# DidItWork/Sigma-Zero

Measured on AMD Instinct MI355X. Metric: MCTS simulations/sec (self-play), higher is better.
Workload: dtype bf16

## Files before the change

### include/sigmazero.h

```cpp
#ifndef SIGMAZERO_H
#define SIGMAZERO_H
#include <stdint.h>

#ifdef __cplusplus
extern "C" {
#endif

#define SZ_RING 256
#define SZ_PLANES 119
#define SZ_ACTIONS 4672
#define SZ_MAX_MOVES 218
#define SZ_POS_BYTES 80

enum {
    SZ_OK = 0,
    SZ_ERR_INVALID = -1,
    SZ_ERR_HIP = -2,
    SZ_ERR_CAPACITY = -3,
    SZ_ERR_NO_DEVICE = -4,
    SZ_ERR_STATE = -5,
    SZ_ERR_ZERO_VISITS = -6
};

enum { SZ_PLANES_F32 = 0, SZ_PLANES_BF16 = 1, SZ_PLANES_NHWC128_BF16 = 2, SZ_PLANES_NHWC128_BITS = 3 };


typedef struct sz_engine sz_engine;

typedef struct sz_config {
    int32_t n_boards;
    int32_t num_searches;
    float   c_puct;
    int32_t learning;
    float   noise_value;
    int32_t chess960;
    int32_t edges_per_board;
    int32_t planes_dtype;
    int32_t device;
    int32_t reuse_subtree;
} sz_config;

typedef struct sz_stats {
    uint64_t simulations;
    uint64_t expansions;
    uint64_t terminal_hits;
    uint64_t sum_depth;
    uint64_t sum_children;
    uint64_t max_edges_used;
    int32_t  boards_pending;
    int32_t  boards_done;
    int32_t  boards_error;
    int32_t  first_error;
} sz_stats;

int sz_create(const sz_config* cfg, sz_engine** out);
int sz_destroy(sz_engine* e);

int sz_new_games(sz_engine* e, const int32_t* scharnagl, const uint8_t* active, void* stream);

int sz_upload_game(sz_engine* e, int32_t board, const void* ring, int32_t ply, void* stream);
int sz_set_active(sz_engine* e, const uint8_t* active, void* stream);

int sz_compact(sz_engine* e, int32_t enable, int32_t* n_live_out, void* stream);

int sz_search_begin(sz_engine* e, void* planes_dev, void* stream);

int sz_search_step(sz_engine* e, const float* policy_dev, const float* value_dev, void* planes_dev, void* stream);

int sz_get_stats(sz_engine* e, sz_stats* out, void* stream);

int sz_root_children(sz_engine* e, int32_t* action_dev, int32_t* visits_dev, int32_t* n_child_dev,
                     float* prior_dev, double* value_sum_dev, void* stream);

int sz_play(sz_engine* e, const double* uniforms_dev, void* stream);

int sz_fetch_ply(sz_engine* e, uint8_t* packed_planes, int32_t* action, int32_t* visits, int32_t* n_child,
                 uint8_t* colour, int32_t* chosen, uint8_t* game_over, int8_t* result, uint8_t* active, void* stream);

int sz_set_root_noise(sz_engine* e, const float* gamma_dev);

int sz_debug_step_stamps(sz_engine* e, void* dev_buffer);

int sz_debug_pending(sz_engine* e, uint64_t* mask, int32_t* depth, int32_t* n_nodes, int32_t* n_edges,
                     int32_t* status, void* stream);
int sz_debug_tree(sz_engine* e, int32_t board, int32_t max_nodes, int32_t* depth, int32_t* action, int32_t* visits, double* value_sum,
                  float* prior, int32_t* n_out, void* stream);
int sz_debug_select(const int32_t* offsets_dev, const int32_t* vc_dev, const double* value_sum_dev, const float* prior_dev,
                    const int32_t* parent_visits_dev, const float* c_dev, float* ucb_out_dev, int32_t* argmax_out_dev, int32_t n_cases, void* stream);
int sz_debug_position(sz_engine* e, int32_t board, void* pos_out, int32_t* ply, void* stream);


int sz_nn_conv_bf16(const void* in, const void* w_packed, const float* bias, const void* residual, void* out,
                    int32_t n_boards, int32_t cin, int32_t ksize, int32_t relu, void* stream);
#define SZ_NN_W16 0x40000
#define SZ_NN_IN_BITS 0x1000000
int sz_nn_block_bf16(const void* in, const void* w1_packed, const float* bias1, const void* w2_packed, const float* bias2, void* out,
                     int32_t n_boards, int32_t flags, void* stream);
int sz_nn_pack_weights(const float* w_in, int32_t cin_real, int32_t cin_padded, int32_t ksize, uint16_t* out);

int sz_nn_pack_weights16(const float* w_in, int32_t cin_real, int32_t cin_padded, int32_t ksize, uint16_t* out);
#define SZ_NN_F16 0x8000000
int sz_nn_pack_weights16_f16(const float* w_in, int32_t cin_real, int32_t cin_padded, int32_t ksize, uint16_t* out);
int sz_nn_pack_head16_f16(const float* w_in, uint16_t* out);

#define SZ_NN_TOWER_WGB1 0x10000000
#define SZ_NN_TOWER_WGB2 0x20000000
int sz_nn_tower_bf16(const void* planes, const void* const* w_packed, const float* const* bias, int32_t n_blocks, void* out,
                     int32_t n_boards, int32_t flags , void* stream);
#define SZ_NN_SPLIT_WGB1 0x2000000
#define SZ_NN_SPLIT_WGB2 0x4000000
int sz_nn_tower_split(const void* planes, const void* w_stream, const float* bias, int32_t n_blocks, float* out,
                      int32_t n_boards, int32_t flags , void* stream);
int64_t sz_nn_split_stream_elems(int32_t n_blocks);
int sz_nn_pack_split_stream(const float* w_in, int32_t cin_real, int32_t ksize , int32_t conv, uint16_t* stream);
int sz_nn_forward_split(const void* planes, const void* w_stream, const float* bias, int32_t n_blocks, const void* w_p2_packed, const float* b_p2,
                        const float* wv, float bv, const float* fc1_w_t, const float* fc1_b, const float* fc2_w, float fc2_b, float* probs, float* value,
                        float* v1_scratch, float* tower_out, int32_t n_boards, int32_t do_softmax, int32_t flags, void* stream);
int sz_nn_pack_split_head(const float* w_in , uint16_t* out);
int sz_nn_pack_split_stream_f16(const float* w_in, int32_t cin_real, int32_t ksize, int32_t conv, uint16_t* stream);
int sz_nn_pack_split_head_f16(const float* w_in, uint16_t* out);
int sz_nn_conv3x3_split_f32(const float* x, const void* w_stream, const float* zero256, float* y, int32_t n_boards, int32_t f16, void* amax_bits, void* stream);
int sz_nn_wgrad3x3_split_f32(const float* gy, const float* x, const void* amax_gy, const void* amax_x, float* part, float* dw, int32_t n_boards, void* stream);
int sz_nn_pack_conv_split_dev(const float* w, int32_t transposed, int32_t f16, void* w_stream, void* zero_u32 , void* stream);
int sz_nn_pack_conv_split_both(const float* w, int32_t f16, void* w_stream, void* w_stream_t, void* zero_u32, void* stream);
int sz_nn_conv3x3_train_fwd(const float* x, const float* w, int32_t f16, void* w_stream, void* w_stream_t, const float* zero256, float* y, int32_t n_boards, void* amax2, void* stream);
int sz_nn_conv3x3_train_bwd(const float* gy, const float* x, const void* w_stream_t, const float* zero256, float* gx, void* amax2, float* part, float* dw, int32_t n_boards,
                            int32_t f16, void* stream);
int sz_bn_act_train_fwd(const float* x, const float* gamma, const float* beta, float* running_mean, float* running_var, float momentum, float eps, const float* residual,
                        float* y, float* save_mean, float* save_invstd, int32_t n_boards, int32_t channels, void* stream);
int sz_bn_act_train_bwd(const float* gy, const float* x, const float* y, const float* gamma, const float* save_mean, const float* save_invstd, float* dx, float* dres,
                        float* dgamma, float* dbeta, int32_t n_boards, int32_t channels, void* stream);
int sz_nn_value_mlp(const float* v1, const float* fc1_w_t, const float* fc1_b, const float* fc2_w, float fc2_b, float* value, int32_t n_boards, void* stream);
int sz_nn_debug_split_stamps(void* dev_buffer, int32_t mode );
int sz_nn_debug_tower_stamps(void* dev_buffer, int32_t mode );
int sz_debug_stream_read(const void* src, uint64_t bytes, int32_t mode, void* sink16, void* stream);
int sz_nn_policy_head_bf16(const void* t, const void* w_packed, const float* bias, float* probs, int32_t n_boards, int32_t do_softmax, void* stream);
int sz_nn_value_head_bf16(const void* x, const float* wv, float bv, const float* fc1_w_t, const float* fc1_b, const float* fc2_w, float fc2_b,
                          float* value, int32_t n_boards, void* stream);
int sz_nn_pack_head16(const float* w_in, uint16_t* out);
int sz_nn_heads_bf16(const void* x, const void* w_p1_packed, const float* b_p1, const void* w_p2_packed, const float* b_p2, const float* wv, float bv,
                     const float* fc1_w_t, const float* fc1_b, const float* fc2_w, float fc2_b, float* probs, float* value, float* v1_scratch,
                     int32_t n_boards, int32_t do_softmax, void* stream);

const char* sz_error_string(int code);
int sz_device_count(void);


typedef struct szh_game szh_game;

szh_game* szh_game_new(int chess960, int scharnagl);
szh_game* szh_game_from_fen(const char* fen, int chess960);
szh_game* szh_game_copy(const szh_game* g);
void      szh_game_free(szh_game* g);
int  szh_legal_actions(const szh_game* g, int32_t* idx);
int  szh_action_to_move(const szh_game* g, int idx, int32_t* from, int32_t* to, int32_t* promo);
int  szh_move_to_action(int from, int to, int promo, int white);
int  szh_push_action(szh_game* g, int idx);
int  szh_push_move(szh_game* g, int from, int to, int promo);
void szh_status(const szh_game* g, int32_t* out12);
void szh_planes(const szh_game* g, uint8_t* out );
uint64_t szh_perft(szh_game* g, int depth);
void szh_bitboards(const szh_game* g, uint64_t* out10);
int  szh_export(const szh_game* g, void* ring_out, int32_t* ply, int32_t* chess960);
int  szh_is_chess960(const szh_game* g);
int  szh_plane_bits_mismatches(const szh_game* g);

#ifdef __cplusplus
}
#endif
#endif
```

### sigma-zero_amd/_native.py

```python
import ctypes as C
import os

from . import build as _build

SZ_RING, SZ_PLANES, SZ_ACTIONS, SZ_MAX_MOVES, SZ_POS_BYTES, SZ_MASK_WORDS = 256, 119, 4672, 218, 80, 73
SZ_OK, SZ_ERR_INVALID, SZ_ERR_HIP, SZ_ERR_CAPACITY, SZ_ERR_NO_DEVICE, SZ_ERR_STATE, SZ_ERR_ZERO_VISITS = 0, -1, -2, -3, -4, -5, -6
SZ_PLANES_F32, SZ_PLANES_BF16, SZ_PLANES_NHWC128_BF16, SZ_PLANES_NHWC128_BITS = 0, 1, 2, 3
SZ_NN_W16 = 0x40000
SZ_NN_IN_BITS = 0x1000000
SZ_NN_SPLIT_WGB1, SZ_NN_SPLIT_WGB2 = 0x2000000, 0x4000000
SZ_NN_F16 = 0x8000000
SZ_NN_TOWER_WGB1, SZ_NN_TOWER_WGB2 = 0x10000000, 0x20000000


class sz_config(C.Structure):
    _fields_ = [("n_boards", C.c_int32), ("num_searches", C.c_int32), ("c_puct", C.c_float), ("learning", C.c_int32),
                ("noise_value", C.c_float), ("chess960", C.c_int32), ("edges_per_board", C.c_int32),
                ("planes_dtype", C.c_int32), ("device", C.c_int32), ("reuse_subtree", C.c_int32)]


class sz_stats(C.Structure):
    _fields_ = [("simulations", C.c_uint64), ("expansions", C.c_uint64), ("terminal_hits", C.c_uint64), ("sum_depth", C.c_uint64),
                ("sum_children", C.c_uint64), ("max_edges_used", C.c_uint64), ("boards_pending", C.c_int32),
                ("boards_done", C.c_int32), ("boards_error", C.c_int32), ("first_error", C.c_int32)]


class NativeError(RuntimeError):
    def __init__(self, code, what=""):
        self.code = code
        msg = lib().sz_error_string(code).decode() if _lib is not None else str(code)
        super().__init__("sigmazero native call failed%s: %s (%d)" % (" in " + what if what else "", msg, code))


EXPORTS = {
    "sz_create": (C.c_int, [C.POINTER(sz_config), C.POINTER(C.c_void_p)]),
    "sz_destroy": (C.c_int, [C.c_void_p]),
    "sz_new_games": (C.c_int, [C.c_void_p, C.c_void_p, C.c_void_p, C.c_void_p]),
    "sz_upload_game": (C.c_int, [C.c_void_p, C.c_int32, C.c_void_p, C.c_int32, C.c_void_p]),
    "sz_set_active": (C.c_int, [C.c_void_p, C.c_void_p, C.c_void_p]),
    "sz_compact": (C.c_int, [C.c_void_p, C.c_int32, C.POINTER(C.c_int32), C.c_void_p]),
    "sz_search_begin": (C.c_int, [C.c_void_p, C.c_void_p, C.c_void_p]),
    "sz_search_step": (C.c_int, [C.c_void_p, C.c_void_p, C.c_void_p, C.c_void_p, C.c_void_p]),
    "sz_get_stats": (C.c_int, [C.c_void_p, C.POINTER(sz_stats), C.c_void_p]),
    "sz_root_children": (C.c_int, [C.c_void_p] + [C.c_void_p] * 5 + [C.c_void_p]),
    "sz_play": (C.c_int, [C.c_void_p, C.c_void_p, C.c_void_p]),
    "sz_fetch_ply": (C.c_int, [C.c_void_p] + [C.c_void_p] * 9 + [C.c_void_p]),
    "sz_debug_pending": (C.c_int, [C.c_void_p] + [C.c_void_p] * 5 + [C.c_void_p]),
    "sz_debug_position": (C.c_int, [C.c_void_p, C.c_int32, C.c_void_p, C.POINTER(C.c_int32), C.c_void_p]),
    "sz_debug_tree": (C.c_int, [C.c_void_p, C.c_int32, C.c_int32] + [C.c_void_p] * 5 + [C.POINTER(C.c_int32), C.c_void_p]),
    "sz_debug_select": (C.c_int, [C.c_void_p] * 8 + [C.c_int32, C.c_void_p]),
    "sz_nn_conv_bf16": (C.c_int, [C.c_void_p] * 5 + [C.c_int32] * 4 + [C.c_void_p]),
    "sz_nn_block_bf16": (C.c_int, [C.c_void_p] * 6 + [C.c_int32] * 2 + [C.c_void_p]),
    "sz_nn_tower_bf16": (C.c_int, [C.c_void_p, C.c_void_p, C.c_void_p, C.c_int32, C.c_void_p, C.c_int32, C.c_int32, C.c_void_p]),
    "sz_nn_tower_split": (C.c_int, [C.c_void_p, C.c_void_p, C.c_void_p, C.c_int32, C.c_void_p, C.c_int32, C.c_int32, C.c_void_p]),
    "sz_nn_debug_split_stamps": (C.c_int, [C.c_void_p, C.c_int32]),
    "sz_nn_split_stream_elems": (C.c_int64, [C.c_int32]),
    "sz_nn_pack_split_stream": (C.c_int, [C.c_void_p, C.c_int32, C.c_int32, C.c_int32, C.c_void_p]),
    "sz_nn_forward_split": (C.c_int, [C.c_void_p, C.c_void_p, C.c_void_p, C.c_int32, C.c_void_p, C.c_void_p, C.c_void_p, C.c_float, C.c_void_p, C.c_void_p, C.c_void_p, C.c_float,
                                      C.c_void_p, C.c_void_p, C.c_void_p, C.c_void_p, C.c_int32, C.c_int32, C.c_int32, C.c_void_p]),
    "sz_nn_pack_split_head": (C.c_int, [C.c_void_p, C.c_void_p]),
    "sz_nn_pack_split_head_f16": (C.c_int, [C.c_void_p, C.c_void_p]),
    "sz_nn_pack_split_stream_f16": (C.c_int, [C.c_void_p, C.c_int32, C.c_int32, C.c_int32, C.c_void_p]),
    "sz_nn_conv3x3_split_f32": (C.c_int, [C.c_void_p, C.c_void_p, C.c_void_p, C.c_void_p, C.c_int32, C.c_int32, C.c_void_p, C.c_void_p]),
    "sz_nn_wgrad3x3_split_f32": (C.c_int, [C.c_void_p, C.c_void_p, C.c_void_p, C.c_void_p, C.c_void_p, C.c_void_p, C.c_int32, C.c_void_p]),
    "sz_nn_pack_conv_split_dev": (C.c_int, [C.c_void_p, C.c_int32, C.c_int32, C.c_void_p, C.c_void_p, C.c_void_p]),
    "sz_nn_pack_conv_split_both": (C.c_int, [C.c_void_p, C.c_int32, C.c_void_p, C.c_void_p, C.c_void_p, C.c_void_p]),
    "sz_bn_act_train_fwd": (C.c_int, [C.c_void_p, C.c_void_p, C.c_void_p, C.c_void_p, C.c_void_p, C.c_float, C.c_float, C.c_void_p, C.c_void_p, C.c_void_p, C.c_void_p, C.c_int32, C.c_int32, C.c_void_p]),
    "sz_bn_act_train_bwd": (C.c_int, [C.c_void_p, C.c_void_p, C.c_void_p, C.c_void_p, C.c_void_p, C.c_void_p, C.c_void_p, C.c_void_p, C.c_void_p, C.c_void_p, C.c_int32, C.c_int32, C.c_void_p]),
    "sz_nn_conv3x3_train_fwd": (C.c_int, [C.c_void_p, C.c_void_p, C.c_int32, C.c_void_p, C.c_void_p, C.c_void_p, C.c_void_p, C.c_int32, C.c_void_p, C.c_void_p]),
    "sz_nn_conv3x3_train_bwd": (C.c_int, [C.c_void_p, C.c_void_p, C.c_void_p, C.c_void_p, C.c_void_p, C.c_void_p, C.c_void_p, C.c_void_p, C.c_int32, C.c_int32, C.c_void_p]),
    "sz_nn_value_mlp": (C.c_int, [C.c_void_p, C.c_void_p, C.c_void_p, C.c_void_p, C.c_float, C.c_void_p, C.c_int32, C.c_void_p]),
    "sz_debug_stream_read": (C.c_int, [C.c_void_p, C.c_uint64, C.c_int32, C.c_void_p, C.c_void_p]),
    "sz_nn_policy_head_bf16": (C.c_int, [C.c_void_p] * 4 + [C.c_int32] * 2 + [C.c_void_p]),
    "sz_debug_step_stamps": (C.c_int, [C.c_void_p, C.c_void_p]),
    "sz_set_root_noise": (C.c_int, [C.c_void_p, C.c_void_p]),
    "sz_nn_debug_tower_stamps": (C.c_int, [C.c_void_p, C.c_int32]),
    "sz_nn_heads_bf16": (C.c_int, [C.c_void_p] * 6 + [C.c_float] + [C.c_void_p] * 3 + [C.c_float] + [C.c_void_p] * 3 + [C.c_int32] * 2 + [C.c_void_p]),
    "sz_nn_value_head_bf16": (C.c_int, [C.c_void_p, C.c_void_p, C.c_float, C.c_void_p, C.c_void_p, C.c_void_p, C.c_float, C.c_void_p, C.c_int32, C.c_void_p]),
    "sz_nn_pack_head16": (C.c_int, [C.c_void_p, C.c_void_p]),
    "sz_nn_pack_head16_f16": (C.c_int, [C.c_void_p, C.c_void_p]),
    "sz_nn_pack_weights16_f16": (C.c_int, [C.c_void_p, C.c_int32, C.c_int32, C.c_int32, C.c_void_p]),
    "sz_nn_pack_weights16": (C.c_int, [C.c_void_p, C.c_int32, C.c_int32, C.c_int32, C.c_void_p]),
    "sz_nn_pack_weights": (C.c_int, [C.c_void_p, C.c_int32, C.c_int32, C.c_int32, C.c_void_p]),
    "sz_error_string": (C.c_char_p, [C.c_int]),
    "sz_device_count": (C.c_int, []),
    "szh_game_new": (C.c_void_p, [C.c_int, C.c_int]),
    "szh_game_from_fen": (C.c_void_p, [C.c_char_p, C.c_int]),
    "szh_game_copy": (C.c_void_p, [C.c_void_p]),
    "szh_game_free": (None, [C.c_void_p]),
    "szh_legal_actions": (C.c_int, [C.c_void_p, C.POINTER(C.c_int32)]),
    "szh_action_to_move": (C.c_int, [C.c_void_p, C.c_int, C.POINTER(C.c_int32), C.POINTER(C.c_int32), C.POINTER(C.c_int32)]),
    "szh_move_to_action": (C.c_int, [C.c_int, C.c_int, C.c_int, C.c_int]),
    "szh_push_action": (C.c_int, [C.c_void_p, C.c_int]),
    "szh_push_move": (C.c_int, [C.c_void_p, C.c_int, C.c_int, C.c_int]),
    "szh_status": (None, [C.c_void_p, C.POINTER(C.c_int32)]),
    "szh_planes": (None, [C.c_void_p, C.c_void_p]),
    "szh_perft": (C.c_uint64, [C.c_void_p, C.c_int]),
    "szh_bitboards": (None, [C.c_void_p, C.POINTER(C.c_uint64)]),
    "szh_export": (C.c_int, [C.c_void_p, C.c_void_p, C.POINTER(C.c_int32), C.POINTER(C.c_int32)]),
    "szh_is_chess960": (C.c_int, [C.c_void_p]),
    "szh_plane_bits_mismatches": (C.c_int, [C.c_void_p]),
}

_lib = None


def lib():
    global _lib
    if _lib is not None:
        return _lib
    path = _build.LIB
    if not os.path.exists(path):
        raise RuntimeError("libsigmazero_hip.so is not built (%s). Run: python -c \"import __graft_entry__ as g; g.build()\". "
                           "The search path has no CPU fallback." % path)
    L = C.CDLL(path)
    for name, (res, args) in EXPORTS.items():
        fn = getattr(L, name)
        fn.restype, fn.argtypes = res, args
    _lib = L
    return L


def check(code, what=""):
    if code != SZ_OK:
        raise NativeError(code, what)
```

### sigma-zero_amd/csrc/sz_nn_split.hip

```cpp
#include "sz_nn_common.h"

#define NN_MAX_CONVS_SPLIT 129
#ifndef SP_PF
#define SP_PF 1
#endif
#define SP_WSCALE_LOG2 10
#ifndef SP_EXPLICIT_WAIT
#define SP_EXPLICIT_WAIT 1
#endif
#define SP_RING (SP_PF == 1 ? 2 : 4)
#define SP_KSTEP_U4 2048

template <int WGB> struct SplitGeom {
    static constexpr int PITCH = NN_COUT * 2 + NN_PAD16;
    static constexpr int IMG = WGB * 64 * PITCH + NN_ZERO16;
    static constexpr int NJ = 4 * WGB;
    static constexpr int TAB = 2 * IMG;
    static constexpr int SCR = 2 * IMG + 9 * NJ * 64 * 4;
    static constexpr int LDS_BYTES = SCR + 1024;
    static constexpr int PITCH_IN = 128 * 2 + NN_PAD16;
};

template <int CIN, int WGB, bool BLO, bool TAB, int ABL = 0 ,
          int NTAPS = 9 ,
          class E = ElemBF16 ,
          int NI = 4 >
__device__ __forceinline__ void split_kloop(const unsigned char* lds, const int offH, const int offL, const int* addr_tab, const WSrc& wr,
                                            const uint32_t ks_base, const uint32_t ks_after, const float* __restrict__ bias,
                                            f32x4 (&acc)[NI][4 * WGB], uint4 (&ring)[SP_RING][2 * NI], const int co_tile0 = -1 ) {
    constexpr int PITCH = CIN * 2 + NN_PAD16;
    constexpr int KSTEPS = CIN / 32;
    constexpr int NJ = 4 * WGB, G = WGB;
    constexpr int NPROD = BLO ? 3 : 2;
    constexpr bool SKIPROWS = WGB == 2 && NN_ROWSKIP && NTAPS == 9;
    static_assert(NTAPS == 9 || NTAPS == 1, "3x3 or 1x1");
    static_assert(KSTEPS % SP_RING == 0, "ring slots must be compile-time indices");
    static_assert(8 + 2 * NI <= NPROD * NI * 3, "every memory instruction needs an MFMA gap of its own");
    int lane = threadIdx.x & 63;
    asm volatile("" : "+v"(lane));
    const int wave = threadIdx.x >> 6;
    const int p16 = lane & 15, kg = lane >> 4;
    const int ct0 = co_tile0 < 0 ? wave * NI : co_tile0;
    const uint32_t wlane = (uint32_t)(ct0 * 64 + lane) * 16u;
    {
        f32x4 binit[NI];
#pragma unroll
        for (int i = 0; i < NI; i++) binit[i] = *(const f32x4*)(bias + (ct0 + i) * 16 + 4 * kg);
#pragma unroll
        for (int i = 0; i < NI; i++)
#pragma unroll
            for (int j = 0; j < NJ; j++) acc[i][j] = binit[i];
    }
    constexpr int TABPITCH = NN_COUT * 2 + NN_PAD16;
    auto tap_addr = [&](int tap, int j) -> int {
        if constexpr (TAB) {
            const int rel = addr_tab[((NTAPS == 1 ? 4 : tap) * NJ + j) * 64 + lane];
            if constexpr (PITCH == TABPITCH) return rel;
            else {
                const int row = (int)__umulhi((unsigned)rel, 7895161u);
                return rel >= WGB * 64 * TABPITCH ? rel - WGB * 64 * (TABPITCH - PITCH) : rel - row * (TABPITCH - PITCH);
            }
        } else return conv_tap_addr16<PITCH, NTAPS, WGB>(tap, j, p16, kg);
    };
    const int lds_base = (int)(uint32_t)(uintptr_t)lds;
    auto abs_addr = [&](int rel) -> int {
        int a = lds_base + offH + rel;
        asm volatile("" : "+v"(a));
        return a;
    };
    auto LD = [](int addr) -> bf16x8 { return *(const __attribute__((address_space(3))) bf16x8*)(uint32_t)addr; };
    int bcurH[NJ], bcurL[BLO ? NJ : 1], bnxt[NJ];
    bf16x8 bH[2][4], bL[4];
#pragma unroll
    for (int j = 0; j < NJ; j++) {
        bnxt[j] = tap_addr(0, j);
        bcurH[j] = abs_addr(bnxt[j]);
        if constexpr (BLO) bcurL[j] = bcurH[j] + (offL - offH);
    }
#pragma unroll
    for (int m = 0; m < 4; m++)
        if (!(SKIPROWS && m == 0)) bH[0][m] = LD(bcurH[m]);
    auto tap_body = [&](const int tap, auto skip_tag) {
        constexpr int SK = decltype(skip_tag)::value;
        if (tap + 1 < NTAPS) {
#pragma unroll
            for (int j = 0; j < NJ; j++) bnxt[j] = tap_addr(tap + 1, j);
        }
#pragma unroll
        for (int kc = 0; kc < KSTEPS; kc++) {
            const int slot = kc & (SP_RING - 1);
            const uint32_t ks_next = (kc + SP_PF >= KSTEPS && tap == NTAPS - 1) ? ks_after + (uint32_t)(kc + SP_PF - KSTEPS) : ks_base + (uint32_t)(tap * KSTEPS + kc + SP_PF);
#pragma unroll
            for (int g = 0; g < G; g++) {
                const int buf = (kc * G + g) & 1;
#pragma unroll
                for (int prod = 0; prod < NPROD; prod++) {
#pragma unroll
                    for (int i = 0; i < NI; i++) {
                        const bf16x8 a = __builtin_bit_cast(bf16x8, ring[slot][prod == 1 ? NI + i : i]);
#pragma unroll
                        for (int m = 0; m < 4; m++) {
                            const bool idle_g = SKIPROWS && ((SK == 1 && g == 0) || (SK == 2 && g == G - 1));
                            const bool idle = idle_g && m == (SK == 1 ? 0 : 3);
                            if (idle) continue;
                            acc[i][g * 4 + m] = E::mfma(a, prod == 2 ? bL[m] : bH[buf][m], acc[i][g * 4 + m]);
                            const int NR = idle_g ? 3 : 4, q = (prod * NI + i) * NR + (idle_g && SK == 1 ? m - 1 : m);
                            if (q < 4) {
                                if constexpr (BLO && !(ABL & 2)) {
                                    const bool idl = SKIPROWS && ((SK == 1 && g == 0 && q == 0) || (SK == 2 && g == G - 1 && q == 3));
                                    if (!idl) bL[q] = LD(bcurL[g * 4 + q] + kc * 64);
                                }
                            } else if (q < 8) {
                                const int mm = q - 4;
                                if (ABL & 2) {
                                } else if (g + 1 < G) {
                                    if (!(SKIPROWS && SK == 2 && g + 1 == G - 1 && mm == 3)) bH[buf ^ 1][mm] = LD(bcurH[(g + 1) * 4 + mm] + kc * 64);
                                } else if (kc + 1 < KSTEPS) {
                                    if (!(SKIPROWS && SK == 1 && mm == 0)) bH[buf ^ 1][mm] = LD(bcurH[mm] + (kc + 1) * 64);
                                } else if (tap + 1 < NTAPS) {
                                    if (!(SKIPROWS && mm == 0 && tap + 1 < 3)) bH[buf ^ 1][mm] = LD(abs_addr(bnxt[mm]));
                                }
                            } else if (q < 8 + 2 * NI && g == 0) {
                                const int f = q - 8;
                                if (!(ABL & 1)) ring[(kc + SP_PF) & (SP_RING - 1)][f] = ld_wfrag(wr, (size_t)ks_next * SP_KSTEP_U4 + (f >= NI ? SP_KSTEP_U4 / 2 : 0), wlane + (f % NI) * 1024);
                            }
#if SP_EXPLICIT_WAIT
                            if (q == 2 * NI * NR - 1 && NPROD == 3) __builtin_amdgcn_s_waitcnt(0xC07F);
                            if (q == NPROD * NI * NR - 1) {
                                if (g == G - 1) __builtin_amdgcn_s_waitcnt(0x0070 | ((SP_PF - 1) * 2 * NI));
                                else __builtin_amdgcn_s_waitcnt(0xC07F);
                            }
#endif
                            asm volatile("" ::: "memory");
                            __builtin_amdgcn_sched_barrier(0);
                        }
                    }
                }
            }
        }
        if (NTAPS > 1) {
#pragma unroll
            for (int j = 0; j < NJ; j++) {
                bcurH[j] = abs_addr(bnxt[j]);
                if constexpr (BLO) bcurL[j] = bcurH[j] + (offL - offH);
            }
        }
    };
    using SK0 = std::integral_constant<int, 0>;
    if constexpr (SKIPROWS) {
        using SK1 = std::integral_constant<int, 1>; using SK2 = std::integral_constant<int, 2>;
        for (int tap = 0; tap < 3; tap++) tap_body(tap, SK1{});
        for (int tap = 3; tap < 6; tap++) tap_body(tap, SK0{});
        for (int tap = 6; tap < 9; tap++) tap_body(tap, SK2{});
    } else {
        for (int tap = 0; tap < NTAPS; tap++) tap_body(tap, SK0{});
    }
}

__device__ __forceinline__ float to_agpr(float v) { float a; asm volatile("v_accvgpr_write_b32 %0, %1" : "=a"(a) : "v"(v)); return a; }
__device__ __forceinline__ float from_agpr(float a) { float v; asm volatile("v_accvgpr_read_b32 %0, %1" : "=v"(v) : "a"(a)); return v; }
__device__ __forceinline__ float relu_f32(float v) { const int i = __builtin_bit_cast(int, v); return __builtin_bit_cast(float, i > 0 ? i : 0); }

template <int WGB, int MODE, class E = ElemBF16>
__device__ __forceinline__ void split_epilogue(unsigned char* hi_img, unsigned char* lo_img, const f32x4 (&acc)[4][4 * WGB], float (&xres)[4][4 * WGB][4]) {
    constexpr bool SCALED = std::is_same<E, ElemF16>::value;
    constexpr float USC = 1.0f / (float)(1 << SP_WSCALE_LOG2);
    constexpr int PITCH = NN_COUT * 2 + NN_PAD16;
    int lane = threadIdx.x & 63;
    asm volatile("" : "+v"(lane));
    const int wave = threadIdx.x >> 6;
    const int p16 = lane & 15, kg = lane >> 4;
#pragma unroll
    for (int j = 0; j < 4 * WGB; j++) {
        const int row = tile_row<WGB>(j, p16);
        const int rowoff = row * PITCH, g = (row >> 2) & 1;
#pragma unroll
        for (int ip = 0; ip < 4; ip += 2) {
            uint2 h[2], l[2];
            float r[2][4];
            f32x4 v[2];
#pragma unroll
            for (int d = 0; d < 2; d++)
#pragma unroll
                for (int k = 0; k < 4; k++) r[d][k] = MODE == 2 ? from_agpr(xres[ip + d][j][k]) : 0.f;
#pragma unroll
            for (int d = 0; d < 2; d++) {
                v[d] = acc[ip + d][j];
#pragma unroll
                for (int k = 0; k < 4; k++) {
                    if (SCALED) v[d][k] *= USC;
                    if (MODE == 2) v[d][k] += r[d][k];
                    v[d][k] = relu_f32(v[d][k]);
                }
            }
#pragma unroll
            for (int d = 0; d < 2; d++)
#pragma unroll
                for (int k = 0; k < 4; k++)
                    if (MODE != 1) xres[ip + d][j][k] = to_agpr(v[d][k]);
#pragma unroll
            for (int d = 0; d < 2; d++) {
                h[d].x = E::pack2(v[d][0], v[d][1]); h[d].y = E::pack2(v[d][2], v[d][3]);
                l[d].x = E::pack2(v[d][0] - E::lo(h[d].x), v[d][1] - E::hi(h[d].x));
                l[d].y = E::pack2(v[d][2] - E::lo(h[d].y), v[d][3] - E::hi(h[d].y));
            }
            const auto hx = __builtin_amdgcn_permlane16_swap(h[0].x, h[1].x, false, false), hy = __builtin_amdgcn_permlane16_swap(h[0].y, h[1].y, false, false);
            const auto lx = __builtin_amdgcn_permlane16_swap(l[0].x, l[1].x, false, false), ly = __builtin_amdgcn_permlane16_swap(l[0].y, l[1].y, false, false);
            const int it = ip + (kg & 1);
            const int chunk = ((wave * 4 + it) * 16 + 4 * (kg & 2)) >> 3;
            const int off = rowoff + ((chunk ^ g) << 4);
            *(uint4*)(hi_img + off) = make_uint4(hx[0], hy[0], hx[1], hy[1]);
            *(uint4*)(lo_img + off) = make_uint4(lx[0], ly[0], lx[1], ly[1]);
        }
    }
}

struct SplitHeadsParams {
    const uint4* w_p2;
    const float* b_p2;
    const float* wv;
    float bv;
    float* probs;
    float* v1_out;
    int do_softmax;
};

template <int WGB, class E = ElemBF16>
__device__ __forceinline__ void split_heads_tail(unsigned char* lds, const int* addr_tab, const WSrc& wr, const uint32_t ks_p1, const float* __restrict__ bias_p1,
                                                 const SplitHeadsParams& hp, f32x4 (&acc)[4][4 * WGB], uint4 (&ring)[SP_RING][8], float (&xres)[4][4 * WGB][4],
                                                 const int board0, const int n_boards) {
    using GEO = SplitGeom<WGB>;
    constexpr int NJ = GEO::NJ, NT = WGB, PITCH = GEO::PITCH;
    unsigned char* imgH = lds;
    unsigned char* imgL = lds + GEO::IMG;
    float* psum = (float*)(lds + GEO::SCR);
    float* red = psum + WGB * 64;
    int lane = threadIdx.x & 63;
    asm volatile("" : "+v"(lane));
    const int wave = threadIdx.x >> 6, p16 = lane & 15, kg = lane >> 4;
    {
        const int row = wave * 64 + lane;
        if (row < WGB * 64) {
            const unsigned char* ph = imgH + row * PITCH;
            const unsigned char* pl = imgL + row * PITCH;
            const int g = (row >> 2) & 1;
            float sv = 0.f;
#pragma unroll 4
            for (int c8 = 0; c8 < 32; c8++) {
                const uint4 h = *(const uint4*)(ph + ((c8 ^ g) << 4)), l = *(const uint4*)(pl + ((c8 ^ g) << 4));
                const float4 w0 = ((const float4*)hp.wv)[c8 * 2], w1 = ((const float4*)hp.wv)[c8 * 2 + 1];
                sv = __builtin_fmaf(w0.x, E::lo(h.x) + E::lo(l.x), sv); sv = __builtin_fmaf(w0.y, E::hi(h.x) + E::hi(l.x), sv);
                sv = __builtin_fmaf(w0.z, E::lo(h.y) + E::lo(l.y), sv); sv = __builtin_fmaf(w0.w, E::hi(h.y) + E::hi(l.y), sv);
                sv = __builtin_fmaf(w1.x, E::lo(h.z) + E::lo(l.z), sv); sv = __builtin_fmaf(w1.y, E::hi(h.z) + E::hi(l.z), sv);
                sv = __builtin_fmaf(w1.z, E::lo(h.w) + E::lo(l.w), sv); sv = __builtin_fmaf(w1.w, E::hi(h.w) + E::hi(l.w), sv);
            }
            const int board = board0 + (row >> 6);
            if (board < n_boards) hp.v1_out[(size_t)board * 64 + (row & 63)] = fmaxf(sv + hp.bv, 0.f);
        }
    }
    split_kloop<256, WGB, true, true, 0, 1, E>(lds, 0, GEO::IMG, addr_tab, wr, ks_p1, 0u, bias_p1, acc, ring);
    __syncthreads();
    split_epilogue<WGB, 1, E>(imgH, imgL, acc, xres);
    __syncthreads();
    f32x4 pa[5][NT];
#pragma unroll
    for (int i = 0; i < 5; i++)
#pragma unroll
        for (int t = 0; t < NT; t++) pa[i][t] = f32x4{0.f, 0.f, 0.f, 0.f};
    int baddr[NT];
#pragma unroll
    for (int t = 0; t < NT; t++) baddr[t] = addr_tab[(4 * NJ + wave * NT + t) * 64 + lane];
#pragma unroll 2
    for (int kc = 0; kc < 8; kc++) {
        bf16x8 ah[5], al[5], bh[NT], bl[NT];
#pragma unroll
        for (int i = 0; i < 5; i++) {
            ah[i] = __builtin_bit_cast(bf16x8, hp.w_p2[(size_t)(kc * 10 + i) * 64 + lane]);
            al[i] = __builtin_bit_cast(bf16x8, hp.w_p2[(size_t)(kc * 10 + 5 + i) * 64 + lane]);
        }
#pragma unroll
        for (int t = 0; t < NT; t++) { bh[t] = *(const bf16x8*)(imgH + baddr[t] + kc * 64); bl[t] = *(const bf16x8*)(imgL + baddr[t] + kc * 64); }
#pragma unroll
        for (int prod = 0; prod < 3; prod++)
#pragma unroll
            for (int i = 0; i < 5; i++)
#pragma unroll
                for (int t = 0; t < NT; t++)
                    pa[i][t] = E::mfma(prod == 1 ? al[i] : ah[i], prod == 2 ? bl[t] : bh[t], pa[i][t]);
    }
    __syncthreads();
    float mx = -3.0e38f;
#pragma unroll
    for (int i = 0; i < 5; i++)
#pragma unroll
        for (int r = 0; r < 4; r++) {
            const int co = i * 16 + 4 * kg + r;
            const float bb = co < 73 ? hp.b_p2[co] : 0.f;
#pragma unroll
            for (int t = 0; t < NT; t++) {
                if (std::is_same<E, ElemF16>::value) pa[i][t][r] *= 1.0f / (float)(1 << SP_WSCALE_LOG2);
                pa[i][t][r] += bb;
                if (co < 73) mx = fmaxf(mx, pa[i][t][r]);
            }
        }
    const int lboard = WGB == 2 ? (p16 >> 3) : 0;
    float inv = 1.0f;
    if (hp.do_softmax) {
        mx = fmaxf(mx, __shfl_xor(mx, 1)); mx = fmaxf(mx, __shfl_xor(mx, 2)); mx = fmaxf(mx, __shfl_xor(mx, 4));
        if (WGB == 1) mx = fmaxf(mx, __shfl_xor(mx, 8));
        mx = fmaxf(mx, __shfl_xor(mx, 16)); mx = fmaxf(mx, __shfl_xor(mx, 32));
        if ((lane & (WGB == 2 ? 0x37 : 0x3F)) == 0) red[wave * 2 + lboard] = mx;
        __syncthreads();
        mx = fmaxf(fmaxf(red[0 + lboard], red[2 + lboard]), fmaxf(red[4 + lboard], red[6 + lboard]));
#pragma unroll
        for (int t = 0; t < NT; t++) {
            float ps = 0.f;
#pragma unroll
            for (int i = 0; i < 5; i++)
#pragma unroll
                for (int r = 0; r < 4; r++) {
                    const int co = i * 16 + 4 * kg + r;
                    const float e = co < 73 ? __expf(pa[i][t][r] - mx) : 0.f;
                    pa[i][t][r] = e;
                    ps += e;
                }
            ps += __shfl_xor(ps, 16);
            ps += __shfl_xor(ps, 32);
            const int row = tile_row<WGB>(wave * NT + t, p16);
            if (kg == 0) psum[row] = ps;
        }
        __syncthreads();
        float tot = 0.f;
#pragma unroll 8
        for (int p = 0; p < 64; p++) tot += psum[lboard * 64 + p];
        inv = 1.0f / tot;
    }
    if (board0 + lboard < n_boards) {
        float* pb = hp.probs + (size_t)(board0 + lboard) * 4672;
#pragma unroll
        for (int t = 0; t < NT; t++) {
            const int pos = tile_row<WGB>(wave * NT + t, p16) & 63;
#pragma unroll
            for (int i = 0; i < 5; i++)
#pragma unroll
                for (int r = 0; r < 4; r++) {
                    const int co = i * 16 + 4 * kg + r;
                    if (co < 73) pb[co * 64 + pos] = pa[i][t][r] * inv;
                }
        }
    }
}

#define SPSTAMP(k) do { if (MODE != 0 && stamp_now) { unsigned long long _t = __builtin_amdgcn_s_memtime(); if ((threadIdx.x & 63) == 0) stamps[(size_t)(blockIdx.x * 4 + (threadIdx.x >> 6)) * 16 + (k)] = _t; } } while (0)
template <int WGB, int MODE, bool HEADS, class E = ElemBF16>
__global__ __launch_bounds__(256, 1) void k_tower_split(const uint16_t* __restrict__ planes, const uint4* __restrict__ wstream, const float* __restrict__ bias,
                                                         float* __restrict__ out, int n_boards, int n_blocks, int flags, unsigned long long* __restrict__ stamps,
                                                         const SplitHeadsParams hp) {
    constexpr int ABL = MODE >= 2 ? MODE - 1 : 0;
    using GEO = SplitGeom<WGB>;
    constexpr int NJ = GEO::NJ;
    extern __shared__ __attribute__((aligned(16))) unsigned char lds[];
    unsigned char* imgH = lds;
    unsigned char* imgL = lds + GEO::IMG;
    for (int c = threadIdx.x; c < NN_ZERO16 / 16; c += 256) {
        *(uint4*)(imgH + WGB * 64 * GEO::PITCH + c * 16) = make_uint4(0, 0, 0, 0);
        *(uint4*)(imgL + WGB * 64 * GEO::PITCH + c * 16) = make_uint4(0, 0, 0, 0);
    }
    int* addr_tab = (int*)(lds + GEO::TAB);
    for (int e = threadIdx.x; e < 9 * NJ * 64; e += 256)
        addr_tab[e] = conv_tap_addr16<GEO::PITCH, 9, WGB, true>(e / (NJ * 64), (e >> 6) % NJ, e & 15, (e >> 4) & 3);
    const int lane = threadIdx.x & 63, wave = threadIdx.x >> 6;
    const int n_tiles = (n_boards + WGB - 1) / WGB;
    const int n_convs = 1 + 2 * n_blocks;
    const WSrc wr = wfrag_rsrc(wstream);
    f32x4 acc[4][NJ];
    float xres[4][NJ][4];
    uint4 ring[SP_RING][8];
    {
        const uint32_t wlane = (uint32_t)((wave * 4) * 64 + lane) * 16u;
#pragma unroll
        for (int k = 0; k < SP_PF; k++)
#pragma unroll
            for (int f = 0; f < 8; f++) ring[k][f] = ld_wfrag(wr, (size_t)k * SP_KSTEP_U4 + (f >= 4 ? SP_KSTEP_U4 / 2 : 0), wlane + (f & 3) * 1024);
    }
    for (int tile = blockIdx.x; tile < n_tiles; tile += gridDim.x) {
        const int board0 = tile * WGB;
        if (flags & SZ_NN_IN_BITS) stage_tile_bits<WGB, NN_PAD16, E, true>(imgL, planes, board0, n_boards);
        else stage_tile<128, WGB, NN_PAD16, false, true>(imgL, planes, board0, n_boards, false);
        __syncthreads();
        uint32_t ks = 0;
        const uint32_t ks_p1 = 36u + 72u * (uint32_t)(n_convs - 1);
        const uint32_t ks_end = HEADS ? ks_p1 : 0u;
        split_kloop<128, WGB, false, true, 0, 9, E>(lds, GEO::IMG, GEO::IMG, addr_tab, wr, ks, n_convs > 1 ? 36u : ks_end, bias, acc, ring);
        ks += 36;
        __syncthreads();
        split_epilogue<WGB, 0, E>(imgH, imgL, acc, xres);
        __syncthreads();
        for (int c = 1; c < n_convs; c++) {
            const bool stamp_now = MODE != 0 && (c == 7 || c == 8) && tile == (int)(blockIdx.x + gridDim.x);
            const int sb = (c & 1) ? 0 : 5;
            SPSTAMP(sb + 0);
            split_kloop<256, WGB, true, true, ABL, 9, E>(lds, 0, GEO::IMG, addr_tab, wr, ks, c + 1 < n_convs ? ks + 72u : ks_end, bias + c * NN_COUT, acc, ring);
            ks += 72;
            SPSTAMP(sb + 1);
            __syncthreads();
            SPSTAMP(sb + 2);
            if (c & 1) split_epilogue<WGB, 1, E>(imgH, imgL, acc, xres);
            else split_epilogue<WGB, 2, E>(imgH, imgL, acc, xres);
            SPSTAMP(sb + 3);
            __syncthreads();
            SPSTAMP(sb + 4);
            if (MODE != 0 && stamp_now && c == 8 && (threadIdx.x & 63) == 0) stamps[(size_t)(blockIdx.x * 4 + (threadIdx.x >> 6)) * 16 + 10] = __builtin_amdgcn_s_memrealtime();
        }
        if constexpr (HEADS) split_heads_tail<WGB, E>(lds, addr_tab, wr, ks_p1, bias + n_convs * NN_COUT, hp, acc, ring, xres, board0, n_boards);
        const int p16 = lane & 15, kg = lane >> 4;
        if (!HEADS || out)
#pragma unroll
        for (int j = 0; j < NJ; j++) {
            const int row = tile_row<WGB>(j, p16);
            if (board0 + (row >> 6) < n_boards) {
                float* dst = out + ((size_t)board0 * 64 + row) * NN_COUT;
#pragma unroll
                for (int i = 0; i < 4; i++)
                    *(f32x4*)(dst + (wave * 4 + i) * 16 + 4 * kg) = f32x4{from_agpr(xres[i][j][0]), from_agpr(xres[i][j][1]), from_agpr(xres[i][j][2]), from_agpr(xres[i][j][3])};
            }
        }
    }
}

#ifndef SZ_CONV_ABL
#define SZ_CONV_ABL 0
#endif
template <class E, int COSPLIT>
__global__ __launch_bounds__(256, 1) void k_conv3x3_split_f32(const float* __restrict__ x, const uint4* __restrict__ wstream, const float* __restrict__ zero_bias,
                                                               float* __restrict__ y, int n_boards, unsigned int* __restrict__ amax_bits ) {
    constexpr int WGB = 1;
    constexpr bool SCALED = std::is_same<E, ElemF16>::value;
    using GEO = SplitGeom<WGB>;
    constexpr int NJ = GEO::NJ, PITCH = GEO::PITCH, NI = 4 / COSPLIT;
    extern __shared__ __attribute__((aligned(16))) unsigned char lds[];
    unsigned char* imgH = lds;
    unsigned char* imgL = lds + GEO::IMG;
    float* wmax = (float*)(lds + GEO::SCR);
    for (int c = threadIdx.x; c < NN_ZERO16 / 16; c += 256) {
        *(uint4*)(imgH + WGB * 64 * PITCH + c * 16) = make_uint4(0, 0, 0, 0);
        *(uint4*)(imgL + WGB * 64 * PITCH + c * 16) = make_uint4(0, 0, 0, 0);
    }
    int* addr_tab = (int*)(lds + GEO::TAB);
    for (int e = threadIdx.x; e < 9 * NJ * 64; e += 256)
        addr_tab[e] = conv_tap_addr16<PITCH, 9, WGB, true>(e / (NJ * 64), (e >> 6) % NJ, e & 15, (e >> 4) & 3);
    const int lane = threadIdx.x & 63, wave = threadIdx.x >> 6;
    const WSrc wr = wfrag_rsrc(wstream);
    f32x4 acc[NI][NJ];
    uint4 ring[SP_RING][2 * NI];
    const int half = COSPLIT == 2 ? (int)(blockIdx.x & 1) : 0, ct0 = half * 8 + wave * NI;
    {
        const uint32_t wlane = (uint32_t)(ct0 * 64 + lane) * 16u;
#pragma unroll
        for (int k = 0; k < SP_PF; k++)
#pragma unroll
            for (int f = 0; f < 2 * NI; f++) ring[k][f] = ld_wfrag(wr, (size_t)k * SP_KSTEP_U4 + (f >= NI ? SP_KSTEP_U4 / 2 : 0), wlane + (f % NI) * 1024);
    }
    for (int board = blockIdx.x / COSPLIT; board < n_boards; board += gridDim.x / COSPLIT) {
        __syncthreads();
        const float4* src = (const float4*)(x + (size_t)board * 256 * 64);
        float4 v[16];
#pragma unroll
        for (int t = 0; t < 16; t++) v[t] = src[(wave + 4 * t) * 64 + lane];
        float sx = 1.f, unscale = 1.f;
        if (SCALED) {
            float m = 0.f;
#pragma unroll
            for (int t = 0; t < 16; t++) m = fmaxf(fmaxf(m, fmaxf(fabsf(v[t].x), fabsf(v[t].y))), fmaxf(fabsf(v[t].z), fabsf(v[t].w)));
            for (int off = 32; off >= 1; off >>= 1) m = fmaxf(m, __shfl_xor(m, off));
            if (lane == 0) wmax[wave] = m;
            __syncthreads();
            m = fmaxf(fmaxf(wmax[0], wmax[1]), fmaxf(wmax[2], wmax[3]));
            if (amax_bits && threadIdx.x == 0 && half == 0) atomicMax(amax_bits, __builtin_bit_cast(unsigned int, m));
            const int ex = (int)((__builtin_bit_cast(uint32_t, m) >> 23) & 0xFF);
            const int k = (ex == 0 || ex == 255) ? 0 : 11 - (ex - 127);
            const int kc = k < -100 ? -100 : (k > 100 ? 100 : k);
            sx = __builtin_bit_cast(float, (uint32_t)(127 + kc) << 23);
            unscale = __builtin_bit_cast(float, (uint32_t)(127 - kc - SP_WSCALE_LOG2) << 23);
        }
#pragma unroll
        for (int t = 0; t < 16; t++) {
            const int q = wave + 4 * t;
            const int c = q * 4 + (lane >> 4), p0 = (lane & 15) * 4;
            const float vv[4] = {v[t].x * sx, v[t].y * sx, v[t].z * sx, v[t].w * sx};
#pragma unroll
            for (int k = 0; k < 4; k++) {
                const int row = p0 + k;
                const int off = row * PITCH + (((c >> 3) ^ ((row >> 2) & 1)) << 4) + (c & 7) * 2;
                const uint32_t hb = E::pack2(vv[k], 0.f) & 0xFFFFu;
                const uint32_t lb = E::pack2(vv[k] - E::lo(hb), 0.f) & 0xFFFFu;
                if (!(SZ_CONV_ABL & 2) || hb == 0x1234u) {
                    *(uint16_t*)(imgH + off) = (uint16_t)hb;
                    *(uint16_t*)(imgL + off) = (uint16_t)lb;
                }
            }
        }
        __syncthreads();
        if (SZ_CONV_ABL & 1) {
#pragma unroll
            for (int i = 0; i < NI; i++)
#pragma unroll
                for (int j = 0; j < NJ; j++) acc[i][j] = f32x4{sx, sx, sx, sx};
        } else
        split_kloop<256, WGB, true, true, 0, 9, E, NI>(lds, 0, GEO::IMG, addr_tab, wr, 0u, 0u, zero_bias, acc, ring, ct0);
        float* dst = y + (size_t)board * 256 * 64;
        const int p16 = lane & 15, kg = lane >> 4;
#pragma unroll
        for (int i = 0; i < NI; i++)
#pragma unroll
            for (int j = 0; j < NJ; j++)
#pragma unroll
                for (int r = 0; r < ((SZ_CONV_ABL & 4) ? 1 : 4); r++) dst[(size_t)((ct0 + i) * 16 + 4 * kg + r) * 64 + j * 16 + p16] = SCALED ? acc[i][j][r] * unscale : acc[i][j][r];
    }
}

template <class E>
__global__ __launch_bounds__(256) void k_pack_conv_split(const float* __restrict__ w, uint16_t* __restrict__ stream, int transposed, unsigned int* __restrict__ zero_u32,
                                                         uint16_t* __restrict__ stream_t ) {
    int idx = blockIdx.x * 256 + threadIdx.x;
    if (zero_u32 && idx == 0) { zero_u32[0] = 0u; if (stream_t) zero_u32[1] = 0u; }
    if (stream_t && idx >= 72 * 16 * 64 * 8) { idx -= 72 * 16 * 64 * 8; stream = stream_t; transposed = 1; }
    if (idx >= 72 * 16 * 64 * 8) return;
    const int e = idx & 7, l = (idx >> 3) & 63, tile = (idx >> 9) & 15, ks = idx >> 13;
    const int tap = ks >> 3, k32 = ks & 7;
    const int co = tile * 16 + (l & 15), ci = k32 * 32 + 8 * (l >> 4) + e;
    float v = transposed ? w[((size_t)ci * 256 + co) * 9 + (8 - tap)] : w[((size_t)co * 256 + ci) * 9 + tap];
    if (std::is_same<E, ElemF16>::value) v *= (float)(1 << SP_WSCALE_LOG2);
    const uint32_t h = E::pack2(v, 0.f) & 0xFFFFu;
    const uint32_t lo = E::pack2(v - E::lo(h), 0.f) & 0xFFFFu;
    uint16_t* rec = stream + (size_t)ks * SP_KSTEP_U4 * 8;
    rec[((size_t)tile * 64 + l) * 8 + e] = (uint16_t)h;
    rec[(size_t)SP_KSTEP_U4 * 4 + ((size_t)tile * 64 + l) * 8 + e] = (uint16_t)lo;
}

#define WG_ROWPITCH 512
#define WG_TILE_BYTES (10 * WG_ROWPITCH)
#define WG_LDS_BYTES (3 * 4 * WG_TILE_BYTES)
__device__ __forceinline__ float pow2_from_amax_bits(unsigned int bits, int target_log2, int* k_out) {
    const int ex = (int)((bits >> 23) & 0xFF);
    int k = (ex == 0 || ex == 255) ? 0 : target_log2 - (ex - 127);
    k = k < -100 ? -100 : (k > 100 ? 100 : k);
    *k_out = k;
    return __builtin_bit_cast(float, (uint32_t)(127 + k) << 23);
}
__global__ __launch_bounds__(256, 1) void k_wgrad3x3_split(const float* __restrict__ gy, const float* __restrict__ x, const unsigned int* __restrict__ amax_gy,
                                                            const unsigned int* __restrict__ amax_x, float* __restrict__ part, int n_boards, int KG) {
    using E = ElemF16;
    extern __shared__ __attribute__((aligned(16))) unsigned char lds[];
    const int cob = blockIdx.x & 3, cib = (blockIdx.x >> 2) & 3, kgrp = blockIdx.x >> 4;
    const int chunk = (n_boards + KG - 1) / KG, b0 = kgrp * chunk, b1 = min(n_boards, b0 + chunk);
    const int lane = threadIdx.x & 63, wave = threadIdx.x >> 6, wr = wave >> 1, wc = wave & 1;
    const int n = lane & 15, kg = lane >> 4;
    int kgy, kx;
    const float sgy = pow2_from_amax_bits(*amax_gy, 11, &kgy), sx = pow2_from_amax_bits(*amax_x, 11, &kx);
    const float unscale_g = __builtin_bit_cast(float, (uint32_t)(127 - kgy) << 23), unscale_x = __builtin_bit_cast(float, (uint32_t)(127 - kx) << 23);
    for (int c = threadIdx.x; c < WG_LDS_BYTES / 16; c += 256) *(uint4*)(lds + c * 16) = make_uint4(0, 0, 0, 0);
    f32x4 acc[2][2][9];
#pragma unroll
    for (int a = 0; a < 2; a++)
#pragma unroll
        for (int c = 0; c < 2; c++)
#pragma unroll
            for (int t = 0; t < 9; t++) acc[a][c][t] = f32x4{0.f, 0.f, 0.f, 0.f};
    const int sci = threadIdx.x & 63, sq = threadIdx.x >> 6;
    const int sbase = (sci >> 4) * WG_TILE_BYTES + (sci & 15) * 16;
    float4 xq[4], gq[2][2][2];
    auto load_board = [&](int bb) {
        const float4* src = (const float4*)(x + ((size_t)bb * 256 + cib * 64 + sci) * 64 + sq * 16);
#pragma unroll
        for (int i = 0; i < 4; i++) xq[i] = src[i];
#pragma unroll
        for (int cot = 0; cot < 2; cot++)
#pragma unroll
            for (int kh = 0; kh < 2; kh++) {
                const int co = cob * 64 + (2 * wr + cot) * 16 + n;
                const float4* g = (const float4*)(gy + ((size_t)bb * 256 + co) * 64 + (4 * kh + kg) * 8);
                gq[cot][kh][0] = g[0]; gq[cot][kh][1] = g[1];
            }
    };
    if (b0 < b1) load_board(b0);
    for (int b = b0; b < b1; b++) {
        __syncthreads();
        {
            const float4 v0 = xq[0], v1 = xq[1], v2 = xq[2], v3 = xq[3];
            const float rows[2][8] = {{v0.x, v0.y, v0.z, v0.w, v1.x, v1.y, v1.z, v1.w}, {v2.x, v2.y, v2.z, v2.w, v3.x, v3.y, v3.z, v3.w}};
#pragma unroll
            for (int rr = 0; rr < 2; rr++) {
                uint32_t h[8], l[8];
#pragma unroll
                for (int c = 0; c < 8; c++) {
                    const float sv = rows[rr][c] * sx;
                    h[c] = E::pack2(sv, 0.f) & 0xFFFFu;
                    l[c] = E::pack2(sv - E::lo(h[c]), 0.f) & 0xFFFFu;
                }
                const int row = 2 * sq + rr + 1;
#pragma unroll
                for (int dxi = 0; dxi < 3; dxi++) {
                    uint32_t ph[4], pl[4];
#pragma unroll
                    for (int p = 0; p < 4; p++) {
                        const int c0 = 2 * p + dxi - 1, c1 = c0 + 1;
                        ph[p] = ((c0 >= 0 && c0 < 8) ? h[c0] : 0u) | (((c1 >= 0 && c1 < 8) ? h[c1] : 0u) << 16);
                        pl[p] = ((c0 >= 0 && c0 < 8) ? l[c0] : 0u) | (((c1 >= 0 && c1 < 8) ? l[c1] : 0u) << 16);
                    }
                    unsigned char* dst = lds + dxi * 4 * WG_TILE_BYTES + sbase + row * WG_ROWPITCH;
                    *(uint4*)dst = make_uint4(ph[0], ph[1], ph[2], ph[3]);
                    *(uint4*)(dst + 256) = make_uint4(pl[0], pl[1], pl[2], pl[3]);
                }
            }
        }
        bf16x8 ah[2][2], al[2][2];
#pragma unroll
        for (int cot = 0; cot < 2; cot++)
#pragma unroll
            for (int kh = 0; kh < 2; kh++) {
                const float4 g0 = gq[cot][kh][0], g1 = gq[cot][kh][1];
                const float f[8] = {g0.x * sgy, g0.y * sgy, g0.z * sgy, g0.w * sgy, g1.x * sgy, g1.y * sgy, g1.z * sgy, g1.w * sgy};
                uint32_t hh[4], ll[4];
#pragma unroll
                for (int p = 0; p < 4; p++) {
                    hh[p] = E::pack2(f[2 * p], f[2 * p + 1]);
                    ll[p] = E::pack2(f[2 * p] - E::lo(hh[p]), f[2 * p + 1] - E::hi(hh[p]));
                }
                ah[cot][kh] = __builtin_bit_cast(bf16x8, make_uint4(hh[0], hh[1], hh[2], hh[3]));
                al[cot][kh] = __builtin_bit_cast(bf16x8, make_uint4(ll[0], ll[1], ll[2], ll[3]));
            }
        if (b + 1 < b1) load_board(b + 1);
        __syncthreads();
        constexpr int WG_AHEAD = 2, NGRP = 36;
        bf16x8 bh[WG_AHEAD + 1], bl[WG_AHEAD + 1];
        auto fetch = [&](int g) {
            const int kh = g / 18, cit = (g / 9) & 1, tap = g % 9, dy = tap / 3 - 1, dxi = tap % 3;
            const unsigned char* src = lds + (dxi * 4 + 2 * wc + cit) * WG_TILE_BYTES + (4 * kh + kg + dy + 1) * WG_ROWPITCH + n * 16;
            bh[g % (WG_AHEAD + 1)] = *(const bf16x8*)src; bl[g % (WG_AHEAD + 1)] = *(const bf16x8*)(src + 256);
        };
#pragma unroll
        for (int g = 0; g < WG_AHEAD; g++) fetch(g);
#pragma unroll
        for (int g = 0; g < NGRP; g++) {
            if (g + WG_AHEAD < NGRP) fetch(g + WG_AHEAD);
            asm volatile("" ::: "memory");
            __builtin_amdgcn_sched_barrier(0);
            const int kh = g / 18, cit = (g / 9) & 1, tap = g % 9, sl = g % (WG_AHEAD + 1);
#pragma unroll
            for (int cot = 0; cot < 2; cot++) {
                acc[cot][cit][tap] = E::mfma(ah[cot][kh], bh[sl], acc[cot][cit][tap]);
                acc[cot][cit][tap] = E::mfma(al[cot][kh], bh[sl], acc[cot][cit][tap]);
                acc[cot][cit][tap] = E::mfma(ah[cot][kh], bl[sl], acc[cot][cit][tap]);
            }
            asm volatile("" ::: "memory");
            __builtin_amdgcn_sched_barrier(0);
        }
    }
#pragma unroll
    for (int cot = 0; cot < 2; cot++)
#pragma unroll
        for (int cit = 0; cit < 2; cit++)
#pragma unroll
            for (int tap = 0; tap < 9; tap++)
#pragma unroll
                for (int r = 0; r < 4; r++) {
                    const int co = cob * 64 + (2 * wr + cot) * 16 + 4 * kg + r, ci = cib * 64 + (2 * wc + cit) * 16 + n;
                    part[(((size_t)kgrp * 9 + tap) * 256 + co) * 256 + ci] = acc[cot][cit][tap][r] * unscale_g * unscale_x;
                }
}
__global__ __launch_bounds__(256) void k_wgrad_reduce(const float* __restrict__ part, float* __restrict__ dw, int KG) {
    const int idx = blockIdx.x * 256 + threadIdx.x;
    float s[9];
#pragma unroll
    for (int t = 0; t < 9; t++) s[t] = 0.f;
    for (int k = 0; k < KG; k++)
#pragma unroll
        for (int t = 0; t < 9; t++) s[t] += part[((size_t)k * 9 + t) * 65536 + idx];
#pragma unroll
    for (int t = 0; t < 9; t++) dw[(size_t)idx * 9 + t] = s[t];
}

static unsigned long long* g_split_stamps = nullptr;
static int g_split_mode = 1;

extern "C" {

int sz_nn_debug_split_stamps(void* dev_buffer, int32_t mode) { g_split_stamps = (unsigned long long*)dev_buffer; g_split_mode = mode; return SZ_OK; }

int64_t sz_nn_split_stream_elems(int32_t n_blocks) {
    if (n_blocks < 0) return SZ_ERR_INVALID;
    return (int64_t)(36 + 72 * 2 * (int64_t)n_blocks + 8) * SP_KSTEP_U4 * 8;
}

static int pack_split_stream_impl(const float* w_in, int32_t cin_real, int32_t ksize, int32_t conv, uint16_t* stream, bool f16);
int sz_nn_pack_split_stream(const float* w_in, int32_t cin_real, int32_t ksize, int32_t conv, uint16_t* stream) { return pack_split_stream_impl(w_in, cin_real, ksize, conv, stream, false); }
int sz_nn_pack_split_stream_f16(const float* w_in, int32_t cin_real, int32_t ksize, int32_t conv, uint16_t* stream) { return pack_split_stream_impl(w_in, cin_real, ksize, conv, stream, true); }
}
static int pack_split_stream_impl(const float* w_in, int32_t cin_real, int32_t ksize, int32_t conv, uint16_t* stream, bool f16) {
    if (!w_in || !stream || conv < 0 || conv > NN_MAX_CONVS_SPLIT || (ksize != 1 && ksize != 3) || (ksize == 1 && !(conv & 1))) return SZ_ERR_INVALID;
    const int cin_padded = conv == 0 ? 128 : 256, taps = ksize * ksize;
    if (cin_real <= 0 || cin_real > cin_padded) return SZ_ERR_INVALID;
    const int ksteps = cin_padded / 32;
    const size_t ks0 = conv == 0 ? 0 : 36 + (size_t)(conv - 1) * 72;
    const float wscale = f16 ? (float)(1 << SP_WSCALE_LOG2) : 1.f;
    auto rne = [f16](float v) -> uint16_t { return f16 ? ElemF16::from_float(v) : ElemBF16::from_float(v); };
    auto back = [f16](uint16_t h) -> float { if (f16) { _Float16 x; memcpy(&x, &h, 2); return (float)x; } const uint32_t hu = (uint32_t)h << 16; float hf; memcpy(&hf, &hu, 4); return hf; };
    for (int t = 0; t < taps; t++)
        for (int k = 0; k < ksteps; k++) {
            uint16_t* rec = stream + (ks0 + (size_t)t * ksteps + k) * SP_KSTEP_U4 * 8;
            for (int tile = 0; tile < 16; tile++)
                for (int l = 0; l < 64; l++)
                    for (int e = 0; e < 8; e++) {
                        const int co = tile * 16 + (l & 15), ci = k * 32 + 8 * (l >> 4) + e;
                        const float v = (ci < cin_real ? w_in[((size_t)co * cin_real + ci) * taps + t] : 0.f) * wscale;
                        const uint16_t h = rne(v);
                        rec[((size_t)tile * 64 + l) * 8 + e] = h;
                        rec[(size_t)SP_KSTEP_U4 * 4 + ((size_t)tile * 64 + l) * 8 + e] = rne(v - back(h));
                    }
        }
    return SZ_OK;
}
extern "C" {

static int pack_split_head_impl(const float* w_in, uint16_t* out, bool f16);
int sz_nn_pack_split_head(const float* w_in, uint16_t* out) { return pack_split_head_impl(w_in, out, false); }
int sz_nn_pack_split_head_f16(const float* w_in, uint16_t* out) { return pack_split_head_impl(w_in, out, true); }
}
static int pack_split_head_impl(const float* w_in, uint16_t* out, bool f16) {
    if (!w_in || !out) return SZ_ERR_INVALID;
    const float wscale = f16 ? (float)(1 << SP_WSCALE_LOG2) : 1.f;
    auto rne = [f16](float v) -> uint16_t { return f16 ? ElemF16::from_float(v) : ElemBF16::from_float(v); };
    auto back = [f16](uint16_t h) -> float { if (f16) { _Float16 x; memcpy(&x, &h, 2); return (float)x; } const uint32_t hu = (uint32_t)h << 16; float hf; memcpy(&hf, &hu, 4); return hf; };
    for (int ks = 0; ks < 8; ks++)
        for (int tile = 0; tile < 5; tile++)
            for (int l = 0; l < 64; l++)
                for (int e = 0; e < 8; e++) {
                    const int co = tile * 16 + (l & 15), ci = ks * 32 + 8 * (l >> 4) + e;
                    const float v = (co < 73 ? w_in[(size_t)co * 256 + ci] : 0.f) * wscale;
                    const uint16_t h = rne(v);
                    out[((((size_t)ks * 2 + 0) * 5 + tile) * 64 + l) * 8 + e] = h;
                    out[((((size_t)ks * 2 + 1) * 5 + tile) * 64 + l) * 8 + e] = rne(v - back(h));
                }
    return SZ_OK;
}
extern "C" {

}

static int launch_split_one(const void* planes, const void* w_stream, const float* bias, int32_t n_blocks, float* out, int32_t n_boards, int32_t flags, void* stream,
                            const SplitHeadsParams* heads);
static int launch_split(const void* planes, const void* w_stream, const float* bias, int32_t n_blocks, float* out, int32_t n_boards, int32_t flags, void* stream,
                        const SplitHeadsParams* heads) {
    const int n_cu = device_cus(), rem = n_boards % (2 * n_cu);
    if (n_boards > 2 * n_cu && rem > 0 && rem <= n_cu && !(flags & (SZ_NN_SPLIT_WGB1 | SZ_NN_SPLIT_WGB2)) && !g_split_stamps) {
        const int head = n_boards - rem;
        const size_t plane_bytes = (flags & SZ_NN_IN_BITS) ? 64 * sizeof(uint4) : (size_t)64 * 128 * 2;
        const int rc = launch_split_one(planes, w_stream, bias, n_blocks, out, head, flags | SZ_NN_SPLIT_WGB2, stream, heads);
        if (rc != SZ_OK) return rc;
        SplitHeadsParams hp2;
        if (heads) { hp2 = *heads; hp2.probs += (size_t)head * 4672; hp2.v1_out += (size_t)head * 64; }
        return launch_split_one((const unsigned char*)planes + head * plane_bytes, w_stream, bias, n_blocks, out ? out + (size_t)head * 64 * 256 : nullptr, rem,
                                flags | SZ_NN_SPLIT_WGB1, stream, heads ? &hp2 : nullptr);
    }
    return launch_split_one(planes, w_stream, bias, n_blocks, out, n_boards, flags, stream, heads);
}
static int launch_split_one(const void* planes, const void* w_stream, const float* bias, int32_t n_blocks, float* out, int32_t n_boards, int32_t flags, void* stream,
                            const SplitHeadsParams* heads) {
    static bool attr_flags[NN_MAX_DEVICES] = {};
    bool& attr_set = attr_flags[current_device_slot()];
    if (!attr_set) {
#define SPLIT_ATTR(W, M, H) HIPCHK(hipFuncSetAttribute((const void*)k_tower_split<W, M, H>, hipFuncAttributeMaxDynamicSharedMemorySize, SplitGeom<W>::LDS_BYTES))
        SPLIT_ATTR(1, 0, false); SPLIT_ATTR(2, 0, false); SPLIT_ATTR(1, 0, true); SPLIT_ATTR(2, 0, true);
        SPLIT_ATTR(2, 1, false); SPLIT_ATTR(2, 2, false); SPLIT_ATTR(2, 3, false); SPLIT_ATTR(2, 4, false);
#undef SPLIT_ATTR
#define SPLIT_ATTR16(W, H) HIPCHK(hipFuncSetAttribute((const void*)k_tower_split<W, 0, H, ElemF16>, hipFuncAttributeMaxDynamicSharedMemorySize, SplitGeom<W>::LDS_BYTES))
        SPLIT_ATTR16(1, false); SPLIT_ATTR16(2, false); SPLIT_ATTR16(1, true); SPLIT_ATTR16(2, true);
#undef SPLIT_ATTR16
        attr_set = true;
    }
    const int n_cu = device_cus();
    const bool one = (flags & SZ_NN_SPLIT_WGB1) || (n_boards <= n_cu && !(flags & SZ_NN_SPLIT_WGB2));
    SplitHeadsParams hp;
    memset(&hp, 0, sizeof hp);
    if (heads) hp = *heads;
    const int n_tiles = one ? n_boards : (n_boards + 1) / 2;
    const dim3 grid(n_tiles < n_cu ? n_tiles : n_cu);
#define SPLIT_LAUNCH(W, M, H, ST) hipLaunchKernelGGL((k_tower_split<W, M, H>), grid, dim3(256), SplitGeom<W>::LDS_BYTES, (hipStream_t)stream, (const uint16_t*)planes, \
                                                     (const uint4*)w_stream, bias, out, n_boards, n_blocks, (int)flags, ST, hp)
#define SPLIT_LAUNCH16(W, H) hipLaunchKernelGGL((k_tower_split<W, 0, H, ElemF16>), grid, dim3(256), SplitGeom<W>::LDS_BYTES, (hipStream_t)stream, (const uint16_t*)planes, \
                                                  (const uint4*)w_stream, bias, out, n_boards, n_blocks, (int)flags, (unsigned long long*)nullptr, hp)
    if (flags & SZ_NN_F16) {
        if (heads) { if (one) SPLIT_LAUNCH16(1, true); else SPLIT_LAUNCH16(2, true); }
        else { if (one) SPLIT_LAUNCH16(1, false); else SPLIT_LAUNCH16(2, false); }
    } else if (heads) {
        if (one) SPLIT_LAUNCH(1, 0, true, (unsigned long long*)nullptr); else SPLIT_LAUNCH(2, 0, true, (unsigned long long*)nullptr);
    } else if (one) SPLIT_LAUNCH(1, 0, false, (unsigned long long*)nullptr);
    else if (!g_split_stamps) SPLIT_LAUNCH(2, 0, false, (unsigned long long*)nullptr);
    else if (g_split_mode == 2) SPLIT_LAUNCH(2, 2, false, g_split_stamps);
    else if (g_split_mode == 3) SPLIT_LAUNCH(2, 3, false, g_split_stamps);
    else if (g_split_mode == 4) SPLIT_LAUNCH(2, 4, false, g_split_stamps);
    else SPLIT_LAUNCH(2, 1, false, g_split_stamps);
#undef SPLIT_LAUNCH
#undef SPLIT_LAUNCH16
    HIPCHK(hipGetLastError());
    return SZ_OK;
}

extern "C" {

int sz_nn_tower_split(const void* planes, const void* w_stream, const float* bias, int32_t n_blocks, float* out, int32_t n_boards, int32_t flags, void* stream) {
    if (!planes || !w_stream || !bias || !out || n_boards <= 0 || n_blocks < 0 || 1 + 2 * n_blocks > NN_MAX_CONVS_SPLIT) return SZ_ERR_INVALID;
    StreamDeviceGuard _guard(stream);
    return launch_split(planes, w_stream, bias, n_blocks, out, n_boards, flags, stream, nullptr);
}

int sz_nn_value_mlp(const float* v1, const float* fc1_w_t, const float* fc1_b, const float* fc2_w, float fc2_b, float* value, int32_t n_boards, void* stream);

int sz_nn_forward_split(const void* planes, const void* w_stream, const float* bias, int32_t n_blocks, const void* w_p2_packed, const float* b_p2, const float* wv, float bv,
                        const float* fc1_w_t, const float* fc1_b, const float* fc2_w, float fc2_b, float* probs, float* value, float* v1_scratch, float* tower_out,
                        int32_t n_boards, int32_t do_softmax, int32_t flags, void* stream) {
    if (!planes || !w_stream || !bias || !w_p2_packed || !b_p2 || !wv || !fc1_w_t || !fc1_b || !fc2_w || !probs || !value || !v1_scratch || n_boards <= 0 || n_blocks < 0 ||
        1 + 2 * n_blocks > NN_MAX_CONVS_SPLIT) return SZ_ERR_INVALID;
    StreamDeviceGuard _guard(stream);
    SplitHeadsParams hp;
    hp.w_p2 = (const uint4*)w_p2_packed; hp.b_p2 = b_p2; hp.wv = wv; hp.bv = bv; hp.probs = probs; hp.v1_out = v1_scratch; hp.do_softmax = do_softmax;
    const int rc = launch_split(planes, w_stream, bias, n_blocks, tower_out, n_boards, flags, stream, &hp);
    if (rc != SZ_OK) return rc;
    return sz_nn_value_mlp(v1_scratch, fc1_w_t, fc1_b, fc2_w, fc2_b, value, n_boards, stream);
}

int sz_nn_conv3x3_split_f32(const float* x, const void* w_stream, const float* zero256, float* y, int32_t n_boards, int32_t f16, void* amax_bits, void* stream) {
    if (!x || !w_stream || !zero256 || !y || n_boards <= 0) return SZ_ERR_INVALID;
    StreamDeviceGuard _guard(stream);
    static bool attr_flags[NN_MAX_DEVICES] = {};
    bool& attr_set = attr_flags[current_device_slot()];
    if (!attr_set) {
        HIPCHK(hipFuncSetAttribute((const void*)k_conv3x3_split_f32<ElemBF16, 1>, hipFuncAttributeMaxDynamicSharedMemorySize, SplitGeom<1>::LDS_BYTES));
        HIPCHK(hipFuncSetAttribute((const void*)k_conv3x3_split_f32<ElemF16, 1>, hipFuncAttributeMaxDynamicSharedMemorySize, SplitGeom<1>::LDS_BYTES));
        HIPCHK(hipFuncSetAttribute((const void*)k_conv3x3_split_f32<ElemBF16, 2>, hipFuncAttributeMaxDynamicSharedMemorySize, SplitGeom<1>::LDS_BYTES));
        HIPCHK(hipFuncSetAttribute((const void*)k_conv3x3_split_f32<ElemF16, 2>, hipFuncAttributeMaxDynamicSharedMemorySize, SplitGeom<1>::LDS_BYTES));
        attr_set = true;
    }
    const int n_cu = device_cus();
    const bool two = 2 * n_boards <= n_cu;
    const dim3 grid(two ? 2 * n_boards : (n_boards < n_cu ? n_boards : n_cu));
#define CONV_LAUNCH(E_, CS_, AM_) hipLaunchKernelGGL((k_conv3x3_split_f32<E_, CS_>), grid, dim3(256), SplitGeom<1>::LDS_BYTES, (hipStream_t)stream, x, (const uint4*)w_stream, zero256, y, n_boards, AM_)
    if (f16) { if (two) CONV_LAUNCH(ElemF16, 2, (unsigned int*)amax_bits); else CONV_LAUNCH(ElemF16, 1, (unsigned int*)amax_bits); }
    else { if (two) CONV_LAUNCH(ElemBF16, 2, (unsigned int*)nullptr); else CONV_LAUNCH(ElemBF16, 1, (unsigned int*)nullptr); }
#undef CONV_LAUNCH
    HIPCHK(hipGetLastError());
    return SZ_OK;
}
int sz_nn_pack_conv_split_dev(const float* w, int32_t transposed, int32_t f16, void* w_stream, void* zero_u32, void* stream) {
    if (!w || !w_stream) return SZ_ERR_INVALID;
    StreamDeviceGuard _guard(stream);
    if (f16) hipLaunchKernelGGL(k_pack_conv_split<ElemF16>, dim3(72 * 16 * 64 * 8 / 256), dim3(256), 0, (hipStream_t)stream, w, (uint16_t*)w_stream, (int)transposed, (unsigned int*)zero_u32, (uint16_t*)nullptr);
    else hipLaunchKernelGGL(k_pack_conv_split<ElemBF16>, dim3(72 * 16 * 64 * 8 / 256), dim3(256), 0, (hipStream_t)stream, w, (uint16_t*)w_stream, (int)transposed, (unsigned int*)zero_u32, (uint16_t*)nullptr);
    HIPCHK(hipGetLastError());
    return SZ_OK;
}
int sz_nn_pack_conv_split_both(const float* w, int32_t f16, void* w_stream, void* w_stream_t, void* zero_u32, void* stream) {
    if (!w || !w_stream || !w_stream_t) return SZ_ERR_INVALID;
    StreamDeviceGuard _guard(stream);
    if (f16) hipLaunchKernelGGL(k_pack_conv_split<ElemF16>, dim3(2 * 72 * 16 * 64 * 8 / 256), dim3(256), 0, (hipStream_t)stream, w, (uint16_t*)w_stream, 0, (unsigned int*)zero_u32, (uint16_t*)w_stream_t);
    else hipLaunchKernelGGL(k_pack_conv_split<ElemBF16>, dim3(2 * 72 * 16 * 64 * 8 / 256), dim3(256), 0, (hipStream_t)stream, w, (uint16_t*)w_stream, 0, (unsigned int*)zero_u32, (uint16_t*)w_stream_t);
    HIPCHK(hipGetLastError());
    return SZ_OK;
}

int sz_nn_wgrad3x3_split_f32(const float* gy, const float* x, const void* amax_gy, const void* amax_x, float* part, float* dw, int32_t n_boards, void* stream) {
    if (!gy || !x || !amax_gy || !amax_x || !part || !dw || n_boards <= 0) return SZ_ERR_INVALID;
    StreamDeviceGuard _guard(stream);
    static bool attr_flags[NN_MAX_DEVICES] = {};
    bool& attr_set = attr_flags[current_device_slot()];
    if (!attr_set) {
        HIPCHK(hipFuncSetAttribute((const void*)k_wgrad3x3_split, hipFuncAttributeMaxDynamicSharedMemorySize, WG_LDS_BYTES));
        attr_set = true;
    }
    const int KG = n_boards < 16 ? n_boards : 16;
    hipLaunchKernelGGL(k_wgrad3x3_split, dim3(16 * KG), dim3(256), WG_LDS_BYTES, (hipStream_t)stream, gy, x, (const unsigned int*)amax_gy, (const unsigned int*)amax_x, part, n_boards, KG);
    hipLaunchKernelGGL(k_wgrad_reduce, dim3(256), dim3(256), 0, (hipStream_t)stream, (const float*)part, dw, KG);
    HIPCHK(hipGetLastError());
    return SZ_OK;
}

int sz_nn_conv3x3_train_fwd(const float* x, const float* w, int32_t f16, void* w_stream, void* w_stream_t, const float* zero256, float* y, int32_t n_boards, void* amax2, void* stream) {
    if (!x || !w || !w_stream || !zero256 || !y || n_boards <= 0) return SZ_ERR_INVALID;
    const int rc = w_stream_t ? sz_nn_pack_conv_split_both(w, f16, w_stream, w_stream_t, amax2, stream) : sz_nn_pack_conv_split_dev(w, 0, f16, w_stream, amax2, stream);
    if (rc != SZ_OK) return rc;
    return sz_nn_conv3x3_split_f32(x, w_stream, zero256, y, n_boards, f16, f16 ? amax2 : nullptr, stream);
}
int sz_nn_conv3x3_train_bwd(const float* gy, const float* x, const void* w_stream_t, const float* zero256, float* gx, void* amax2, float* part, float* dw, int32_t n_boards,
                            int32_t f16, void* stream) {
    if (!gy || n_boards <= 0 || (!gx && !dw)) return SZ_ERR_INVALID;
    if (gx) {
        if (!w_stream_t || !zero256) return SZ_ERR_INVALID;
        const int rc = sz_nn_conv3x3_split_f32(gy, w_stream_t, zero256, gx, n_boards, f16, (f16 && amax2) ? (void*)((unsigned int*)amax2 + 1) : nullptr, stream);
        if (rc != SZ_OK) return rc;
    }
    if (dw) {
        if (!x || !amax2 || !part || !f16) return SZ_ERR_INVALID;
        return sz_nn_wgrad3x3_split_f32(gy, x, (const unsigned int*)amax2 + 1, amax2, part, dw, n_boards, stream);
    }
    return SZ_OK;
}

}
```

### sigma-zero_amd/fastnet.py

```python
import ctypes as C

import numpy as np
import torch

from . import _native as N


def _fold_bn(conv_w, bn, conv_b=None):
    scale = bn.weight.detach().double() / torch.sqrt(bn.running_var.detach().double() + bn.eps)
    w = conv_w.detach().double() * scale.view(-1, 1, 1, 1)
    b = bn.bias.detach().double() - bn.running_mean.detach().double() * scale
    if conv_b is not None:
        b = b + conv_b.detach().double() * scale
    return w.float(), b.float()


def _pack(w, cin_padded, ksize, device, w16=False, f16=False):
    w = w.contiguous().cpu().float().numpy()
    co, cin = w.shape[0], w.shape[1]
    assert co == 256 and (w16 or not f16)
    out = np.zeros(ksize * ksize * cin_padded * 256, dtype=np.uint16)
    fn = (N.lib().sz_nn_pack_weights16_f16 if f16 else N.lib().sz_nn_pack_weights16) if w16 else N.lib().sz_nn_pack_weights
    N.check(fn(w.ctypes.data_as(C.c_void_p), cin, cin_padded, ksize, out.ctypes.data_as(C.c_void_p)), "sz_nn_pack_weights")
    return torch.from_numpy(out.view(np.int16)).to(device)


class FastPolicyNet:

    def __init__(self, model, device=None, mfma16=True, operands="bf16"):
        model = model.eval()
        assert operands in ("bf16", "fp16") and (operands == "bf16" or mfma16)
        self.operands = operands
        self.f16 = operands == "fp16"
        self.eflag = N.SZ_NN_F16 if self.f16 else 0
        self.force_wgb = 0
        if device is None:
            pdev = next(model.parameters()).device
            device = pdev if pdev.type == "cuda" else torch.device("cuda", torch.cuda.current_device())
        self.device = torch.device(device)
        if self.device.index is None:
            self.device = torch.device("cuda", torch.cuda.current_device())
        dev = self.device
        self.w16 = bool(mfma16)
        self.flag = N.SZ_NN_W16 if self.w16 else 0
        pack_fn = _pack
        def _pack_w(w, cin_padded, ksize, device):
            return pack_fn(w, cin_padded, ksize, device, w16=self.w16, f16=self.f16)
        self.layers = []
        w, b = _fold_bn(model.conv1.weight, model.norm_layer)
        self.stem = (_pack_w(w, 128, 3, dev), b.to(dev).contiguous())
        self.blocks = []
        for blk in model.resnet_blocks:
            w1, b1 = _fold_bn(blk.conv1.weight, blk.bn1)
            w2, b2 = _fold_bn(blk.conv2.weight, blk.bn2)
            self.blocks.append((_pack_w(w1, 256, 3, dev), b1.to(dev).contiguous(), _pack_w(w2, 256, 3, dev), b2.to(dev).contiguous()))
        wp, bp = _fold_bn(model.conv_p1.weight, model.p_norm1)
        self.p1 = (_pack_w(wp, 256, 1, dev), bp.to(dev).contiguous())
        self.wp2 = model.conv_p2.weight.detach().view(73, 256).t().contiguous().to(dev).to(torch.bfloat16)
        self.bp2 = model.conv_p2.bias.detach().float().to(dev)
        wv, bv = _fold_bn(model.conv_v1.weight, model.v_norm)
        self.wv = wv.view(1, 256).t().contiguous().to(dev).to(torch.bfloat16)
        self.bv = bv.to(dev)
        self.fc1_w = model.fc_v1.weight.detach().float().t().contiguous().to(dev)
        self.fc1_b = model.fc_v1.bias.detach().float().to(dev)
        self.fc2_w = model.fc_v2.weight.detach().float().t().contiguous().to(dev)
        self.fc2_b = model.fc_v2.bias.detach().float().to(dev)
        wp2 = model.conv_p2.weight.detach().view(73, 256).contiguous().cpu().float().numpy()
        packed = np.zeros(8 * 5 * 64 * 8, dtype=np.uint16)
        N.check((N.lib().sz_nn_pack_head16_f16 if self.f16 else N.lib().sz_nn_pack_head16)(wp2.ctypes.data_as(C.c_void_p), packed.ctypes.data_as(C.c_void_p)), "sz_nn_pack_head16")
        self.wp2_packed = torch.from_numpy(packed.view(np.int16)).to(dev)
        self.wv_f32 = wv.view(256).contiguous().to(dev)
        self.bv_f = float(bv.view(-1)[0])
        self.fc2_w_vec = self.fc2_w.view(256).contiguous()
        self.fc2_b_f = float(self.fc2_b.view(-1)[0])
        self.native_heads = True
        self.fused_heads = self.w16
        self.persistent_tower = self.w16
        self.persistent_max_boards = 1 << 30
        if self.w16:
            ws = [self.stem[0]] + [w for blk in self.blocks for w in (blk[0], blk[2])]
            bs = [self.stem[1]] + [b for blk in self.blocks for b in (blk[1], blk[3])]
            self._tower_w = (C.c_void_p * len(ws))(*[t.data_ptr() for t in ws])
            self._tower_b = (C.c_void_p * len(bs))(*[t.data_ptr() for t in bs])
        self._bufs, self._full, self._cap = {}, None, 0
        self.fuse_blocks = True
        self.timing = None

    def parameters(self):
        return iter([self.wp2])

    def to(self, *a, **k):
        return self

    def _buffers(self, B):
        if B > self._cap:
            dev = self.device
            self._full = [torch.empty(B, 64, 256, dtype=torch.bfloat16, device=dev) for _ in range(3)] + \
                         [torch.empty(B, 4672, dtype=torch.float32, device=dev), torch.empty(B, dtype=torch.float32, device=dev),
                          torch.empty(B, 64, dtype=torch.float32, device=dev)]
            self._cap = B
            self._bufs = {}
        if B not in self._bufs:
            if len(self._bufs) > 64:
                self._bufs = {}
            self._bufs[B] = [t[:B] for t in self._full]
        return self._bufs[B]

    def _conv(self, x, w, b, res, out, B, cin, ksize, relu=1):
        ev = None
        if self.timing is not None and cin == 256 and ksize == 3 and not self.fuse_blocks:
            ev = (torch.cuda.Event(enable_timing=True), torch.cuda.Event(enable_timing=True))
            ev[0].record()
        self._launch(x, w, b, res, out, B, cin, ksize, relu)
        if ev is not None:
            ev[1].record()
            self.timing.append(ev)

    def _launch(self, x, w, b, res, out, B, cin, ksize, relu):
        N.check(N.lib().sz_nn_conv_bf16(C.c_void_p(x.data_ptr()), C.c_void_p(w.data_ptr()), C.c_void_p(b.data_ptr()),
                                        C.c_void_p(res.data_ptr()) if res is not None else None, C.c_void_p(out.data_ptr()),
                                        B, cin, ksize, relu | self.flag, C.c_void_p(torch.cuda.current_stream(self.device).cuda_stream)), "sz_nn_conv_bf16")

    @torch.no_grad()
    def tower(self, planes):
        B = planes.shape[0]
        a, t, c = self._buffers(B)[:3]
        in_bits = N.SZ_NN_IN_BITS if planes.dtype == torch.uint8 else 0
        if self.f16 and planes.dtype == torch.bfloat16:
            planes = planes.to(torch.float16)
        if in_bits and not self.w16:
            raise ValueError("bit-packed planes need the 16x16x32 kernels (mfma16=True)")
        if self.persistent_tower and (B <= self.persistent_max_boards):
            ev = None
            if self.timing is not None:
                ev = (torch.cuda.Event(enable_timing=True), torch.cuda.Event(enable_timing=True))
                ev[0].record()
            N.check(N.lib().sz_nn_tower_bf16(C.c_void_p(planes.data_ptr()), self._tower_w, self._tower_b, len(self.blocks), C.c_void_p(a.data_ptr()), B, in_bits | self.eflag | self.force_wgb,
                                             C.c_void_p(torch.cuda.current_stream(self.device).cuda_stream)), "sz_nn_tower_bf16")
            if ev is not None:
                ev[1].record()
                self.timing.append(ev)
            return a, t
        if self.f16:
            raise ValueError("fp16 operands need the persistent tower")
        self._conv(planes, self.stem[0], self.stem[1], None, a, B, 128, 3, relu=1 | in_bits)
        for (w1, b1, w2, b2) in self.blocks:
            if self.fuse_blocks:
                self._block(a, w1, b1, w2, b2, c, B)
            else:
                self._conv(a, w1, b1, None, t, B, 256, 3)
                self._conv(t, w2, b2, a, c, B, 256, 3)
            a, c = c, a
        return a, t

    def _block(self, x, w1, b1, w2, b2, out, B):
        ev = None
        if self.timing is not None:
            ev = (torch.cuda.Event(enable_timing=True), torch.cuda.Event(enable_timing=True))
            ev[0].record()
        N.check(N.lib().sz_nn_block_bf16(C.c_void_p(x.data_ptr()), C.c_void_p(w1.data_ptr()), C.c_void_p(b1.data_ptr()), C.c_void_p(w2.data_ptr()),
                                         C.c_void_p(b2.data_ptr()), C.c_void_p(out.data_ptr()), B, self.flag,
                                         C.c_void_p(torch.cuda.current_stream(self.device).cuda_stream)), "sz_nn_block_bf16")
        if ev is not None:
            ev[1].record()
            self.timing.append(ev)

    @torch.no_grad()
    def __call__(self, planes, inference=True):
        if torch.cuda.current_device() != self.device.index:
            with torch.cuda.device(self.device):
                return self._forward(planes, inference)
        return self._forward(planes, inference)

    def _forward(self, planes, inference=True):
        B = planes.shape[0]
        x, scratch = self.tower(planes)
        if self.native_heads:
            policy, value, v1 = self._buffers(B)[3:6]
            st = C.c_void_p(torch.cuda.current_stream(self.device).cuda_stream)
            if self.fused_heads and self.w16:
                P = lambda t: C.c_void_p(t.data_ptr())
                N.check(N.lib().sz_nn_heads_bf16(P(x), P(self.p1[0]), P(self.p1[1]), P(self.wp2_packed), P(self.bp2), P(self.wv_f32), self.bv_f,
                                                 P(self.fc1_w), P(self.fc1_b), P(self.fc2_w_vec), self.fc2_b_f, P(policy), P(value), P(v1),
                                                 B, int(bool(inference)) | self.eflag, st), "sz_nn_heads_bf16")
                return policy, value.view(B, 1)
            if self.f16:
                raise ValueError("fp16 operands need the fused heads")
            self._conv(x, self.p1[0], self.p1[1], None, scratch, B, 256, 1)
            N.check(N.lib().sz_nn_policy_head_bf16(C.c_void_p(scratch.data_ptr()), C.c_void_p(self.wp2_packed.data_ptr()), C.c_void_p(self.bp2.data_ptr()),
                                                   C.c_void_p(policy.data_ptr()), B, int(bool(inference)), st), "sz_nn_policy_head_bf16")
            N.check(N.lib().sz_nn_value_head_bf16(C.c_void_p(x.data_ptr()), C.c_void_p(self.wv_f32.data_ptr()), self.bv_f, C.c_void_p(self.fc1_w.data_ptr()),
                                                  C.c_void_p(self.fc1_b.data_ptr()), C.c_void_p(self.fc2_w_vec.data_ptr()), self.fc2_b_f,
                                                  C.c_void_p(value.data_ptr()), B, st), "sz_nn_value_head_bf16")
            return policy, value.view(B, 1)
        self._conv(x, self.p1[0], self.p1[1], None, scratch, B, 256, 1)
        logits = torch.matmul(scratch.view(B * 64, 256), self.wp2).float().view(B, 64, 73) + self.bp2
        logits = logits.transpose(1, 2).reshape(B, 73 * 64)
        policy = torch.softmax(logits, dim=1) if inference else logits
        v = torch.relu(torch.matmul(x.view(B * 64, 256), self.wv).float().view(B, 64) + self.bv)
        v = torch.relu(v @ self.fc1_w + self.fc1_b)
        value = torch.tanh(v @ self.fc2_w + self.fc2_b)
        return policy, value


def planes_nchw_to_nhwc128(planes):
    B = planes.shape[0]
    out = torch.zeros(B, 64, 128, dtype=torch.bfloat16, device=planes.device)
    out[:, :, :119] = planes.reshape(B, 119, 64).transpose(1, 2).to(torch.bfloat16)
    return out


class SplitPolicyNet:

    def __init__(self, model, device=None, operands="bf16"):
        model = model.eval()
        assert operands in ("bf16", "fp16")
        self.operands, self.f16 = operands, operands == "fp16"
        if device is None:
            pdev = next(model.parameters()).device
            device = pdev if pdev.type == "cuda" else torch.device("cuda", torch.cuda.current_device())
        self.device = torch.device(device)
        if self.device.index is None:
            self.device = torch.device("cuda", torch.cuda.current_device())
        dev = self.device
        self.model = model.to(dev).float()
        self.w16 = True
        convs = [_fold_bn(model.conv1.weight, model.norm_layer)]
        for blk in model.resnet_blocks:
            convs.append(_fold_bn(blk.conv1.weight, blk.bn1))
            convs.append(_fold_bn(blk.conv2.weight, blk.bn2))
        self.n_blocks = len(model.resnet_blocks)
        L = N.lib()
        stream = np.zeros(int(L.sz_nn_split_stream_elems(self.n_blocks)), dtype=np.uint16)
        wp1, bp1 = _fold_bn(model.conv_p1.weight, model.p_norm1)
        for k, (w, b) in enumerate(convs + [(wp1, bp1)]):
            wk = w.contiguous().cpu().float().numpy()
            assert wk.shape[0] == 256 and wk.shape[2] == wk.shape[3] == (1 if k == len(convs) else 3)
            N.check((L.sz_nn_pack_split_stream_f16 if self.f16 else L.sz_nn_pack_split_stream)(wk.ctypes.data_as(C.c_void_p), wk.shape[1], wk.shape[2], k,
                                                                                             stream.ctypes.data_as(C.c_void_p)), "sz_nn_pack_split_stream")
        self._wstream = torch.from_numpy(stream.view(np.int16)).to(dev)
        self._bias = (torch.stack([b for _, b in convs] + [bp1]).float() * (1024.0 if self.f16 else 1.0)).contiguous().to(dev)
        self._eflag = N.SZ_NN_F16 if self.f16 else 0
        self.force_wgb = 0
        wp2 = model.conv_p2.weight.detach().view(73, 256).contiguous().cpu().float().numpy()
        p2 = np.zeros(8 * 2 * 5 * 64 * 8, dtype=np.uint16)
        N.check((L.sz_nn_pack_split_head_f16 if self.f16 else L.sz_nn_pack_split_head)(wp2.ctypes.data_as(C.c_void_p), p2.ctypes.data_as(C.c_void_p)), "sz_nn_pack_split_head")
        self._wp2 = torch.from_numpy(p2.view(np.int16)).to(dev)
        self.fused_heads = True
        self._hbuf, self._hcap = None, 0
        self.h_wp1, self.h_bp1 = wp1.view(256, 256).t().contiguous().to(dev), bp1.to(dev)
        self.h_wp2, self.h_bp2 = model.conv_p2.weight.detach().float().view(73, 256).t().contiguous().to(dev), model.conv_p2.bias.detach().float().to(dev)
        wv, bv = _fold_bn(model.conv_v1.weight, model.v_norm)
        self.h_wv, self.h_bv = wv.view(1, 256).t().contiguous().to(dev), bv.to(dev)
        self._wv_vec, self._bv_f = wv.view(256).contiguous().to(dev), float(bv.view(-1)[0])
        self.h_fc1_w, self.h_fc1_b = model.fc_v1.weight.detach().float().t().contiguous().to(dev), model.fc_v1.bias.detach().float().to(dev)
        self.h_fc2_w, self.h_fc2_b = model.fc_v2.weight.detach().float().t().contiguous().to(dev), model.fc_v2.bias.detach().float().to(dev)
        self._fc2_vec, self._fc2_b_f = self.h_fc2_w.view(256).contiguous(), float(self.h_fc2_b.view(-1)[0])
        self.module_heads = False
        self._out, self._cap = None, 0
        self._p = torch.zeros(1, dtype=torch.float32, device=dev)
        self.timing = None

    def parameters(self):
        return iter([self._p])

    def to(self, *a, **k):
        return self

    def eval(self):
        return self

    @torch.no_grad()
    def tower(self, planes):
        B = planes.shape[0]
        if B > self._cap:
            self._out, self._cap = torch.empty(B, 64, 256, dtype=torch.float32, device=self.device), B
        out = self._out[:B]
        flags = (N.SZ_NN_IN_BITS if planes.dtype == torch.uint8 else 0) | self.force_wgb | self._eflag
        if self.f16 and planes.dtype == torch.bfloat16:
            planes = planes.to(torch.float16)
        ev = None
        if self.timing is not None:
            ev = (torch.cuda.Event(enable_timing=True), torch.cuda.Event(enable_timing=True))
            ev[0].record()
        N.check(N.lib().sz_nn_tower_split(C.c_void_p(planes.data_ptr()), C.c_void_p(self._wstream.data_ptr()), C.c_void_p(self._bias.data_ptr()), self.n_blocks,
                                          C.c_void_p(out.data_ptr()), B, flags, C.c_void_p(torch.cuda.current_stream(self.device).cuda_stream)), "sz_nn_tower_split")
        if ev is not None:
            ev[1].record()
            self.timing.append(ev)
        return out

    @torch.no_grad()
    def __call__(self, planes, inference=True):
        if torch.cuda.current_device() != self.device.index:
            with torch.cuda.device(self.device):
                return self._forward(planes, inference)
        return self._forward(planes, inference)

    def _forward(self, planes, inference=True):
        B = planes.shape[0]
        if self.fused_heads and not self.module_heads:
            if B > self._hcap:
                self._hbuf = (torch.empty(B, 4672, dtype=torch.float32, device=self.device), torch.empty(B, dtype=torch.float32, device=self.device),
                              torch.empty(B, 64, dtype=torch.float32, device=self.device))
                self._hcap = B
            policy, value, v1 = (t[:B] for t in self._hbuf)
            P = lambda t: C.c_void_p(t.data_ptr())
            flags = (N.SZ_NN_IN_BITS if planes.dtype == torch.uint8 else 0) | self.force_wgb | self._eflag
            if self.f16 and planes.dtype == torch.bfloat16:
                planes = planes.to(torch.float16)
            ev = None
            if self.timing is not None:
                ev = (torch.cuda.Event(enable_timing=True), torch.cuda.Event(enable_timing=True))
                ev[0].record()
            N.check(N.lib().sz_nn_forward_split(P(planes), P(self._wstream), P(self._bias), self.n_blocks, P(self._wp2), P(self.h_bp2), P(self._wv_vec), self._bv_f,
                                                P(self.h_fc1_w), P(self.h_fc1_b), P(self._fc2_vec), self._fc2_b_f, P(policy), P(value), P(v1), None,
                                                B, int(bool(inference)), flags, C.c_void_p(torch.cuda.current_stream(self.device).cuda_stream)), "sz_nn_forward_split")
            if ev is not None:
                ev[1].record()
                self.timing.append(ev)
            return policy, value.view(B, 1)
        out = self.tower(planes)
        if self.module_heads:
            x = out.view(B, 8, 8, 256).permute(0, 3, 1, 2)
            policy, value = self.model.policy_head(x), self.model.value_head(x)
        else:
            x2 = out.view(B * 64, 256)
            t = torch.relu(torch.addmm(self.h_bp1, x2, self.h_wp1))
            policy = torch.addmm(self.h_bp2, t, self.h_wp2).view(B, 64, 73).transpose(1, 2).reshape(B, 73 * 64)
            v = torch.relu(torch.addmm(self.h_bv, x2, self.h_wv)).view(B, 64)
            value = torch.tanh(torch.addmm(self.h_fc2_b, torch.relu(torch.addmm(self.h_fc1_b, v, self.h_fc1_w)), self.h_fc2_w))
        if inference:
            policy = torch.softmax(policy, dim=1)
        return policy, value
```

Baseline: 571,200.

## Add mixed f16+fp8 split-precision tower path and make it the default

Adds a split-precision mode for the residual tower in which the low-order residual half of activations and weights is held in scaled fp8 (e4m3) rather than a second f16 word, and is multiplied with the MX-scaled 16x16x128 fp8 MFMA. The high part stays f16. New host packers build the fp8 weight stream and policy-head weights with per-conv scale codes, and the epilogue and value head pack and unpack fp8 low parts. The goal is to halve the work and bytes spent on the correction term. The cost is some accuracy in the residual correction, plus extra permlane transposes and conversions in the epilogue.

Result: no change. 571,000, median of 6 (-0.0%).

```diff
diff --git a/include/sigmazero.h b/include/sigmazero.h
--- a/include/sigmazero.h
+++ b/include/sigmazero.h
@@ -119,6 +119,11 @@
 int sz_nn_pack_split_head(const float* w_in , uint16_t* out);
 int sz_nn_pack_split_stream_f16(const float* w_in, int32_t cin_real, int32_t ksize, int32_t conv, uint16_t* stream);
 int sz_nn_pack_split_head_f16(const float* w_in, uint16_t* out);
+#define SZ_NN_SPLIT_F8 0x40000000
+int64_t sz_nn_split_stream_f8_bytes(int32_t n_blocks);
+int sz_nn_pack_split_stream_f8(const float* w_in, int32_t cin_real, int32_t ksize, int32_t conv, int32_t n_blocks, void* stream);
+int64_t sz_nn_split_head_f8_bytes(void);
+int sz_nn_pack_split_head_f8(const float* w_in , void* out);
 int sz_nn_conv3x3_split_f32(const float* x, const void* w_stream, const float* zero256, float* y, int32_t n_boards, int32_t f16, void* amax_bits, void* stream);
 int sz_nn_wgrad3x3_split_f32(const float* gy, const float* x, const void* amax_gy, const void* amax_x, float* part, float* dw, int32_t n_boards, void* stream);
 int sz_nn_pack_conv_split_dev(const float* w, int32_t transposed, int32_t f16, void* w_stream, void* zero_u32 , void* stream);
diff --git a/sigma-zero_amd/_native.py b/sigma-zero_amd/_native.py
--- a/sigma-zero_amd/_native.py
+++ b/sigma-zero_amd/_native.py
@@ -10,6 +10,7 @@
 SZ_NN_IN_BITS = 0x1000000
 SZ_NN_SPLIT_WGB1, SZ_NN_SPLIT_WGB2 = 0x2000000, 0x4000000
 SZ_NN_F16 = 0x8000000
+SZ_NN_SPLIT_F8 = 0x40000000
 SZ_NN_TOWER_WGB1, SZ_NN_TOWER_WGB2 = 0x10000000, 0x20000000
 
 
@@ -61,6 +62,10 @@
     "sz_nn_pack_split_head": (C.c_int, [C.c_void_p, C.c_void_p]),
     "sz_nn_pack_split_head_f16": (C.c_int, [C.c_void_p, C.c_void_p]),
     "sz_nn_pack_split_stream_f16": (C.c_int, [C.c_void_p, C.c_int32, C.c_int32, C.c_int32, C.c_void_p]),
+    "sz_nn_split_stream_f8_bytes": (C.c_int64, [C.c_int32]),
+    "sz_nn_pack_split_stream_f8": (C.c_int, [C.c_void_p, C.c_int32, C.c_int32, C.c_int32, C.c_int32, C.c_void_p]),
+    "sz_nn_split_head_f8_bytes": (C.c_int64, []),
+    "sz_nn_pack_split_head_f8": (C.c_int, [C.c_void_p, C.c_void_p]),
     "sz_nn_conv3x3_split_f32": (C.c_int, [C.c_void_p, C.c_void_p, C.c_void_p, C.c_void_p, C.c_int32, C.c_int32, C.c_void_p, C.c_void_p]),
     "sz_nn_wgrad3x3_split_f32": (C.c_int, [C.c_void_p, C.c_void_p, C.c_void_p, C.c_void_p, C.c_void_p, C.c_void_p, C.c_int32, C.c_void_p]),
     "sz_nn_pack_conv_split_dev": (C.c_int, [C.c_void_p, C.c_int32, C.c_int32, C.c_void_p, C.c_void_p, C.c_void_p]),
diff --git a/sigma-zero_amd/csrc/sz_nn_split.hip b/sigma-zero_amd/csrc/sz_nn_split.hip
--- a/sigma-zero_amd/csrc/sz_nn_split.hip
+++ b/sigma-zero_amd/csrc/sz_nn_split.hip
@@ -1,4 +1,5 @@
 #include "sz_nn_common.h"
+#include <cmath>
 
 #define NN_MAX_CONVS_SPLIT 129
 #ifndef SP_PF
@@ -157,13 +158,166 @@
     }
 }
 
+struct ElemF16F8 : ElemF16 {};
+#define SP_F8_XLO_LOG2 11
+#define SP_HEAD_F8_U4 (4 * 4 * 5 * 64)
+typedef __attribute__((ext_vector_type(4))) int i32x4;
+typedef __attribute__((ext_vector_type(8))) int i32x8;
+typedef __attribute__((ext_vector_type(2))) short i16x2s;
+__device__ __forceinline__ f32x4 mfma_f8(const i32x4 a0, const i32x4 a1, const i32x4 b0, const i32x4 b1, const f32x4 c, const int sa) {
+    const i32x8 a = __builtin_shufflevector(a0, a1, 0, 1, 2, 3, 4, 5, 6, 7), b = __builtin_shufflevector(b0, b1, 0, 1, 2, 3, 4, 5, 6, 7);
+    return __builtin_amdgcn_mfma_scale_f32_16x16x128_f8f6f4(a, b, c, 0 , 0 , 0, sa, 0, 127 );
+}
+__device__ __forceinline__ uint32_t pack4_fp8(float a, float b, float c, float d) {
+    i16x2s w = {0, 0};
+    w = __builtin_amdgcn_cvt_scalef32_pk_fp8_f32(w, a, b, 1.0f, false);
+    w = __builtin_amdgcn_cvt_scalef32_pk_fp8_f32(w, c, d, 1.0f, true);
+    return __builtin_bit_cast(uint32_t, w);
+}
+template <bool HI> __device__ __forceinline__ f32x2 unpack2_fp8(uint32_t w) { return __builtin_amdgcn_cvt_scalef32_pk_f32_fp8(w, 1.0f, HI); }
+
+template <int WGB, int NTAPS = 9>
+__device__ __forceinline__ void split_kloop_f8(const unsigned char* lds, const int offH, const int offF, const int* addr_tab, const WSrc& wr,
+                                               const uint32_t ks_base, const uint32_t ks_after, const float* __restrict__ bias,
+                                               f32x4 (&acc)[4][4 * WGB], uint4 (&ring)[SP_RING][8], const int sa) {
+    constexpr int NI = 4, NB = 4;
+    constexpr int NJ = 4 * WGB, G = WGB;
+    constexpr bool SKIPROWS = WGB == 2 && NN_ROWSKIP && NTAPS == 9;
+    static_assert(SP_PF == 1 && SP_RING == 2, "the f16 + fp8 loop alternates hi / fp8 records in ring slots 0 / 1");
+    static_assert(NTAPS == 9 || NTAPS == 1, "3x3 or 1x1");
+    int lane = threadIdx.x & 63;
+    asm volatile("" : "+v"(lane));
+    const int wave = threadIdx.x >> 6;
+    const int kg = lane >> 4;
+    const int ct0 = wave * NI;
+    const uint32_t wlane = (uint32_t)(ct0 * 64 + lane) * 16u;
+    {
+        f32x4 binit[NI];
+#pragma unroll
+        for (int i = 0; i < NI; i++) binit[i] = *(const f32x4*)(bias + (ct0 + i) * 16 + 4 * kg);
+#pragma unroll
+        for (int i = 0; i < NI; i++)
+#pragma unroll
+            for (int j = 0; j < NJ; j++) acc[i][j] = binit[i];
+    }
+    auto tap_addr = [&](int tap, int j) -> int { return addr_tab[((NTAPS == 1 ? 4 : tap) * NJ + j) * 64 + lane]; };
+    const int lds_base = (int)(uint32_t)(uintptr_t)lds;
+    auto abs_addr = [&](int rel) -> int {
+        int a = lds_base + offH + rel;
+        asm volatile("" : "+v"(a));
+        return a;
+    };
+    auto LD = [](int addr) -> i32x4 { return *(const __attribute__((address_space(3))) i32x4*)(uint32_t)addr; };
+    const int dF = offF - offH;
+    int bcur[NJ], bnxt[NJ];
+    i32x4 bb[2][8];
+#pragma unroll
+    for (int j = 0; j < NJ; j++) {
+        bnxt[j] = tap_addr(0, j);
+        bcur[j] = abs_addr(bnxt[j]);
+    }
+    auto frag_addr = [&](const int* base, int m, int s, int g, int r) -> int {
+        return s == 0 ? base[g * 4 + (r & 3)] + (2 * m + (r >> 2)) * 64 : base[g * 4 + (r >> 1)] + dF + (2 * m + (r & 1)) * 64;
+    };
+    auto frag_tile = [](int s, int r) { return s == 0 ? (r & 3) : (r >> 1); };
+#pragma unroll
+    for (int r = 0; r < 8; r++)
+        if (!(SKIPROWS && frag_tile(0, r) == 0)) bb[0][r] = LD(frag_addr(bcur, 0, 0, 0, r));
+    auto tap_body = [&](const int tap, auto skip_tag) {
+        constexpr int SK = decltype(skip_tag)::value;
+        if (tap + 1 < NTAPS) {
+#pragma unroll
+            for (int j = 0; j < NJ; j++) bnxt[j] = tap_addr(tap + 1, j);
+        }
+#pragma unroll
+        for (int m = 0; m < NB; m++) {
+#pragma unroll
+            for (int s = 0; s < 2; s++) {
+                const bool last_rec = m == NB - 1 && s == 1;
+                const uint32_t ks_next = (last_rec && tap == NTAPS - 1) ? ks_after : ks_base + (uint32_t)(tap * 2 * NB + 2 * m + s + 1);
+#pragma unroll
+                for (int g = 0; g < G; g++) {
+                    const int buf = ((2 * m + s) * G + g) & 1;
+                    const bool idle_g = SKIPROWS && ((SK == 1 && g == 0) || (SK == 2 && g == G - 1));
+                    const int idle_m = SK == 1 ? 0 : 3;
+                    const int NR = idle_g ? 3 : 4;
+                    const int NMF = (s == 0 ? 2 * NI : NI) * NR;
+                    const bool nx_same_tap = g + 1 < G || s == 0 || m + 1 < NB;
+                    const int nm = g + 1 < G ? m : (s == 0 ? m : m + 1), ns = g + 1 < G ? s : (s ^ 1), ng = g + 1 < G ? g + 1 : 0;
+                    const bool nx_idle_g = SKIPROWS && nx_same_tap && ((SK == 1 && ng == 0) || (SK == 2 && ng == G - 1));
+                    auto mem = [&](const int q) {
+                        if (q < 8) {
+                            const int r = q;
+                            if (nx_same_tap) {
+                                if (!(nx_idle_g && frag_tile(ns, r) == idle_m)) bb[buf ^ 1][r] = LD(frag_addr(bcur, nm, ns, ng, r));
+                            } else if (tap + 1 < NTAPS) {
+                                if (!(SKIPROWS && frag_tile(0, r) == 0 && tap + 1 < 3)) bb[buf ^ 1][r] = LD(abs_addr(bnxt[r & 3]) + (r >> 2) * 64);
+                            }
+                        }
+                        const int qw = (NMF >= 16 ? 8 : NMF - 8);
+                        if (g == 0 && q >= qw && q < qw + 8) {
+                            const int f = q - qw;
+                            ring[s ^ 1][f] = ld_wfrag(wr, (size_t)ks_next * SP_KSTEP_U4 + (f >= 4 ? SP_KSTEP_U4 / 2 : 0), wlane + (f & 3) * 1024);
+                        }
+#if SP_EXPLICIT_WAIT
+                        if (q == NMF - 1) {
+                            if (g == G - 1) __builtin_amdgcn_s_waitcnt(0x0070);
+                            else __builtin_amdgcn_s_waitcnt(0xC07F);
+                        }
+#endif
+                        asm volatile("" ::: "memory");
+                        __builtin_amdgcn_sched_barrier(0);
+                    };
+                    if (s == 0) {
+#pragma unroll
+                        for (int k = 0; k < 2; k++)
+#pragma unroll
+                            for (int i = 0; i < NI; i++)
+#pragma unroll
+                                for (int mm = 0; mm < 4; mm++) {
+                                    if (idle_g && mm == idle_m) continue;
+                                    acc[i][g * 4 + mm] = ElemF16::mfma(__builtin_bit_cast(bf16x8, ring[0][k * 4 + i]), __builtin_bit_cast(bf16x8, bb[buf][k * 4 + mm]), acc[i][g * 4 + mm]);
+                                    mem((k * NI + i) * NR + (idle_g && SK == 1 ? mm - 1 : mm));
+                                }
+                    } else {
+#pragma unroll
+                        for (int mm = 0; mm < 4; mm++) {
+                            if (idle_g && mm == idle_m) continue;
+#pragma unroll
+                            for (int i = 0; i < NI; i++) {
+                                acc[i][g * 4 + mm] = mfma_f8(__builtin_bit_cast(i32x4, ring[1][i]), __builtin_bit_cast(i32x4, ring[1][4 + i]), bb[buf][2 * mm], bb[buf][2 * mm + 1],
+                                                             acc[i][g * 4 + mm], sa);
+                                mem((idle_g && SK == 1 ? mm - 1 : mm) * NI + i);
+                            }
+                        }
+                    }
+                }
+            }
+        }
+        if (NTAPS > 1) {
+#pragma unroll
+            for (int j = 0; j < NJ; j++) bcur[j] = abs_addr(bnxt[j]);
+        }
+    };
+    using SK0 = std::integral_constant<int, 0>;
+    if constexpr (SKIPROWS) {
+        using SK1 = std::integral_constant<int, 1>; using SK2 = std::integral_constant<int, 2>;
+        for (int tap = 0; tap < 3; tap++) tap_body(tap, SK1{});
+        for (int tap = 3; tap < 6; tap++) tap_body(tap, SK0{});
+        for (int tap = 6; tap < 9; tap++) tap_body(tap, SK2{});
+    } else {
+        for (int tap = 0; tap < NTAPS; tap++) tap_body(tap, SK0{});
+    }
+}
+
 __device__ __forceinline__ float to_agpr(float v) { float a; asm volatile("v_accvgpr_write_b32 %0, %1" : "=a"(a) : "v"(v)); return a; }
 __device__ __forceinline__ float from_agpr(float a) { float v; asm volatile("v_accvgpr_read_b32 %0, %1" : "=v"(v) : "a"(a)); return v; }
 __device__ __forceinline__ float relu_f32(float v) { const int i = __builtin_bit_cast(int, v); return __builtin_bit_cast(float, i > 0 ? i : 0); }
 
 template <int WGB, int MODE, class E = ElemBF16>
 __device__ __forceinline__ void split_epilogue(unsigned char* hi_img, unsigned char* lo_img, const f32x4 (&acc)[4][4 * WGB], float (&xres)[4][4 * WGB][4]) {
-    constexpr bool SCALED = std::is_same<E, ElemF16>::value;
+    constexpr bool F8 = std::is_same<E, ElemF16F8>::value;
+    constexpr bool SCALED = std::is_same<E, ElemF16>::value || F8;
     constexpr float USC = 1.0f / (float)(1 << SP_WSCALE_LOG2);
     constexpr int PITCH = NN_COUT * 2 + NN_PAD16;
     int lane = threadIdx.x & 63;
@@ -174,6 +328,7 @@
     for (int j = 0; j < 4 * WGB; j++) {
         const int row = tile_row<WGB>(j, p16);
         const int rowoff = row * PITCH, g = (row >> 2) & 1;
+        uint32_t w8l[4], w8h[4];
 #pragma unroll
         for (int ip = 0; ip < 4; ip += 2) {
             uint2 h[2], l[2];
@@ -201,16 +356,37 @@
 #pragma unroll
             for (int d = 0; d < 2; d++) {
                 h[d].x = E::pack2(v[d][0], v[d][1]); h[d].y = E::pack2(v[d][2], v[d][3]);
-                l[d].x = E::pack2(v[d][0] - E::lo(h[d].x), v[d][1] - E::hi(h[d].x));
-                l[d].y = E::pack2(v[d][2] - E::lo(h[d].y), v[d][3] - E::hi(h[d].y));
+                if constexpr (F8) {
+                    constexpr float LS = (float)(1 << SP_F8_XLO_LOG2), MX = 448.f;
+                    auto lo8 = [&](float vv, float hh) { return __builtin_amdgcn_fmed3f((vv - hh) * LS, -MX, MX); };
+                    w8l[ip + d] = pack4_fp8(lo8(v[d][0], E::lo(h[d].x)), lo8(v[d][1], E::hi(h[d].x)), lo8(v[d][2], E::lo(h[d].y)), lo8(v[d][3], E::hi(h[d].y)));
+                    w8h[ip + d] = pack4_fp8(fminf(v[d][0], MX), fminf(v[d][1], MX), fminf(v[d][2], MX), fminf(v[d][3], MX));
+                } else {
+                    l[d].x = E::pack2(v[d][0] - E::lo(h[d].x), v[d][1] - E::hi(h[d].x));
+                    l[d].y = E::pack2(v[d][2] - E::lo(h[d].y), v[d][3] - E::hi(h[d].y));
+                }
             }
             const auto hx = __builtin_amdgcn_permlane16_swap(h[0].x, h[1].x, false, false), hy = __builtin_amdgcn_permlane16_swap(h[0].y, h[1].y, false, false);
-            const auto lx = __builtin_amdgcn_permlane16_swap(l[0].x, l[1].x, false, false), ly = __builtin_amdgcn_permlane16_swap(l[0].y, l[1].y, false, false);
             const int it = ip + (kg & 1);
             const int chunk = ((wave * 4 + it) * 16 + 4 * (kg & 2)) >> 3;
             const int off = rowoff + ((chunk ^ g) << 4);
             *(uint4*)(hi_img + off) = make_uint4(hx[0], hy[0], hx[1], hy[1]);
-            *(uint4*)(lo_img + off) = make_uint4(lx[0], ly[0], lx[1], ly[1]);
+            if constexpr (!F8) {
+                const auto lx = __builtin_amdgcn_permlane16_swap(l[0].x, l[1].x, false, false), ly = __builtin_amdgcn_permlane16_swap(l[0].y, l[1].y, false, false);
+                *(uint4*)(lo_img + off) = make_uint4(lx[0], ly[0], lx[1], ly[1]);
+            }
+        }
+        if constexpr (F8) {
+            auto transpose4 = [](uint32_t (&w)[4]) {
+                auto a = __builtin_amdgcn_permlane32_swap(w[0], w[2], false, false), b = __builtin_amdgcn_permlane32_swap(w[1], w[3], false, false);
+                auto c = __builtin_amdgcn_permlane16_swap(a[0], b[0], false, false), d = __builtin_amdgcn_permlane16_swap(a[1], b[1], false, false);
+                w[0] = c[0]; w[1] = c[1]; w[2] = d[0]; w[3] = d[1];
+            };
+            transpose4(w8l);
+            transpose4(w8h);
+            const int clo = 8 * wave + kg, chi = 8 * wave + 4 + kg;
+            *(uint4*)(lo_img + rowoff + ((clo ^ g) << 4)) = make_uint4(w8l[0], w8l[1], w8l[2], w8l[3]);
+            *(uint4*)(lo_img + rowoff + ((chi ^ g) << 4)) = make_uint4(w8h[0], w8h[1], w8h[2], w8h[3]);
         }
     }
 }
@@ -228,9 +404,10 @@
 template <int WGB, class E = ElemBF16>
 __device__ __forceinline__ void split_heads_tail(unsigned char* lds, const int* addr_tab, const WSrc& wr, const uint32_t ks_p1, const float* __restrict__ bias_p1,
                                                  const SplitHeadsParams& hp, f32x4 (&acc)[4][4 * WGB], uint4 (&ring)[SP_RING][8], float (&xres)[4][4 * WGB][4],
-                                                 const int board0, const int n_boards) {
+                                                 const int board0, const int n_boards, const int sa_p1 = 0 ) {
     using GEO = SplitGeom<WGB>;
     constexpr int NJ = GEO::NJ, NT = WGB, PITCH = GEO::PITCH;
+    constexpr bool F8 = std::is_same<E, ElemF16F8>::value;
     unsigned char* imgH = lds;
     unsigned char* imgL = lds + GEO::IMG;
     float* psum = (float*)(lds + GEO::SCR);
@@ -245,6 +422,23 @@
             const unsigned char* pl = imgL + row * PITCH;
             const int g = (row >> 2) & 1;
             float sv = 0.f;
+            if constexpr (F8) {
+#pragma unroll 2
+                for (int c16 = 0; c16 < 16; c16++) {
+                    const int m = c16 >> 2, q = c16 & 3;
+                    const uint4 h0 = *(const uint4*)(ph + (((2 * c16) ^ g) << 4)), h1 = *(const uint4*)(ph + (((2 * c16 + 1) ^ g) << 4));
+                    const uint4 l8 = *(const uint4*)(pl + (((8 * m + q) ^ g) << 4));
+                    const uint32_t hw[8] = {h0.x, h0.y, h0.z, h0.w, h1.x, h1.y, h1.z, h1.w}, lw[4] = {l8.x, l8.y, l8.z, l8.w};
+                    const float* wv = hp.wv + c16 * 16;
+#pragma unroll
+                    for (int e = 0; e < 16; e += 2) {
+                        const f32x2 lo = (e & 2) ? unpack2_fp8<true>(lw[e >> 2]) : unpack2_fp8<false>(lw[e >> 2]);
+                        constexpr float ILS = 1.0f / (float)(1 << SP_F8_XLO_LOG2);
+                        sv = __builtin_fmaf(wv[e], ElemF16::lo(hw[e >> 1]) + lo[0] * ILS, sv);
+                        sv = __builtin_fmaf(wv[e + 1], ElemF16::hi(hw[e >> 1]) + lo[1] * ILS, sv);
+                    }
+                }
+            } else
 #pragma unroll 4
             for (int c8 = 0; c8 < 32; c8++) {
                 const uint4 h = *(const uint4*)(ph + ((c8 ^ g) << 4)), l = *(const uint4*)(pl + ((c8 ^ g) << 4));
@@ -258,7 +452,8 @@
             if (board < n_boards) hp.v1_out[(size_t)board * 64 + (row & 63)] = fmaxf(sv + hp.bv, 0.f);
         }
     }
-    split_kloop<256, WGB, true, true, 0, 1, E>(lds, 0, GEO::IMG, addr_tab, wr, ks_p1, 0u, bias_p1, acc, ring);
+    if constexpr (F8) split_kloop_f8<WGB, 1>(lds, 0, GEO::IMG, addr_tab, wr, ks_p1, 0u, bias_p1, acc, ring, sa_p1);
+    else split_kloop<256, WGB, true, true, 0, 1, E>(lds, 0, GEO::IMG, addr_tab, wr, ks_p1, 0u, bias_p1, acc, ring);
     __syncthreads();
     split_epilogue<WGB, 1, E>(imgH, imgL, acc, xres);
     __syncthreads();
@@ -270,6 +465,36 @@
     int baddr[NT];
 #pragma unroll
     for (int t = 0; t < NT; t++) baddr[t] = addr_tab[(4 * NJ + wave * NT + t) * 64 + lane];
+    if constexpr (F8) {
+        const int sa_p2 = (int)*(const uint32_t*)(hp.w_p2 + SP_HEAD_F8_U4);
+#pragma unroll 1
+        for (int m = 0; m < 4; m++) {
+#pragma unroll
+            for (int k = 0; k < 2; k++) {
+                bf16x8 ah[5], bh[NT];
+#pragma unroll
+                for (int i = 0; i < 5; i++) ah[i] = __builtin_bit_cast(bf16x8, hp.w_p2[(size_t)((m * 4 + k) * 5 + i) * 64 + lane]);
+#pragma unroll
+                for (int t = 0; t < NT; t++) bh[t] = *(const bf16x8*)(imgH + baddr[t] + (2 * m + k) * 64);
+#pragma unroll
+                for (int i = 0; i < 5; i++)
+#pragma unroll
+                    for (int t = 0; t < NT; t++) pa[i][t] = ElemF16::mfma(ah[i], bh[t], pa[i][t]);
+            }
+            i32x4 a0[5], a1[5], b0[NT], b1[NT];
+#pragma unroll
+            for (int i = 0; i < 5; i++) {
+                a0[i] = __builtin_bit_cast(i32x4, hp.w_p2[(size_t)((m * 4 + 2) * 5 + i) * 64 + lane]);
+                a1[i] = __builtin_bit_cast(i32x4, hp.w_p2[(size_t)((m * 4 + 3) * 5 + i) * 64 + lane]);
+            }
+#pragma unroll
+            for (int t = 0; t < NT; t++) { b0[t] = *(const i32x4*)(imgL + baddr[t] + (2 * m) * 64); b1[t] = *(const i32x4*)(imgL + baddr[t] + (2 * m + 1) * 64); }
+#pragma unroll
+            for (int i = 0; i < 5; i++)
+#pragma unroll
+                for (int t = 0; t < NT; t++) pa[i][t] = mfma_f8(a0[i], a1[i], b0[t], b1[t], pa[i][t], sa_p2);
+        }
+    } else
 #pragma unroll 2
     for (int kc = 0; kc < 8; kc++) {
         bf16x8 ah[5], al[5], bh[NT], bl[NT];
@@ -298,7 +523,7 @@
             const float bb = co < 73 ? hp.b_p2[co] : 0.f;
 #pragma unroll
             for (int t = 0; t < NT; t++) {
-                if (std::is_same<E, ElemF16>::value) pa[i][t][r] *= 1.0f / (float)(1 << SP_WSCALE_LOG2);
+                if (std::is_same<E, ElemF16>::value || F8) pa[i][t][r] *= 1.0f / (float)(1 << SP_WSCALE_LOG2);
                 pa[i][t][r] += bb;
                 if (co < 73) mx = fmaxf(mx, pa[i][t][r]);
             }
@@ -357,6 +582,8 @@
                                                          float* __restrict__ out, int n_boards, int n_blocks, int flags, unsigned long long* __restrict__ stamps,
                                                          const SplitHeadsParams hp) {
     constexpr int ABL = MODE >= 2 ? MODE - 1 : 0;
+    constexpr bool F8 = std::is_same<E, ElemF16F8>::value;
+    using ES = typename std::conditional<F8, ElemF16, E>::type;
     using GEO = SplitGeom<WGB>;
     constexpr int NJ = GEO::NJ;
     extern __shared__ __attribute__((aligned(16))) unsigned char lds[];
@@ -373,6 +600,7 @@
     const int n_tiles = (n_boards + WGB - 1) / WGB;
     const int n_convs = 1 + 2 * n_blocks;
     const WSrc wr = wfrag_rsrc(wstream);
+    const uint32_t* f8_scale = (const uint32_t*)(wstream + (size_t)(36 + 72 * (n_convs - 1) + 8) * SP_KSTEP_U4);
     f32x4 acc[4][NJ];
     float xres[4][NJ][4];
     uint4 ring[SP_RING][8];
@@ -391,7 +619,7 @@
         uint32_t ks = 0;
         const uint32_t ks_p1 = 36u + 72u * (uint32_t)(n_convs - 1);
         const uint32_t ks_end = HEADS ? ks_p1 : 0u;
-        split_kloop<128, WGB, false, true, 0, 9, E>(lds, GEO::IMG, GEO::IMG, addr_tab, wr, ks, n_convs > 1 ? 36u : ks_end, bias, acc, ring);
+        split_kloop<128, WGB, false, true, 0, 9, ES>(lds, GEO::IMG, GEO::IMG, addr_tab, wr, ks, n_convs > 1 ? 36u : ks_end, bias, acc, ring);
         ks += 36;
         __syncthreads();
         split_epilogue<WGB, 0, E>(imgH, imgL, acc, xres);
@@ -400,7 +628,8 @@
             const bool stamp_now = MODE != 0 && (c == 7 || c == 8) && tile == (int)(blockIdx.x + gridDim.x);
             const int sb = (c & 1) ? 0 : 5;
             SPSTAMP(sb + 0);
-            split_kloop<256, WGB, true, true, ABL, 9, E>(lds, 0, GEO::IMG, addr_tab, wr, ks, c + 1 < n_convs ? ks + 72u : ks_end, bias + c * NN_COUT, acc, ring);
+            if constexpr (F8) split_kloop_f8<WGB, 9>(lds, 0, GEO::IMG, addr_tab, wr, ks, c + 1 < n_convs ? ks + 72u : ks_end, bias + c * NN_COUT, acc, ring, (int)f8_scale[c]);
+            else split_kloop<256, WGB, true, true, ABL, 9, E>(lds, 0, GEO::IMG, addr_tab, wr, ks, c + 1 < n_convs ? ks + 72u : ks_end, bias + c * NN_COUT, acc, ring);
             ks += 72;
             SPSTAMP(sb + 1);
             __syncthreads();
@@ -412,7 +641,8 @@
             SPSTAMP(sb + 4);
             if (MODE != 0 && stamp_now && c == 8 && (threadIdx.x & 63) == 0) stamps[(size_t)(blockIdx.x * 4 + (threadIdx.x >> 6)) * 16 + 10] = __builtin_amdgcn_s_memrealtime();
         }
-        if constexpr (HEADS) split_heads_tail<WGB, E>(lds, addr_tab, wr, ks_p1, bias + n_convs * NN_COUT, hp, acc, ring, xres, board0, n_boards);
+        if constexpr (HEADS) split_heads_tail<WGB, E>(lds, addr_tab, wr, ks_p1, bias + n_convs * NN_COUT, hp, acc, ring, xres, board0, n_boards,
+                                                                 F8 ? (int)f8_scale[n_convs] : 0);
         const int p16 = lane & 15, kg = lane >> 4;
         if (!HEADS || out)
 #pragma unroll
@@ -721,7 +951,97 @@
         }
     return SZ_OK;
 }
+static uint8_t host_e4m3(float v) {
+    const uint8_t sgn = (std::signbit(v) ? 0x80u : 0u);
+    const float a = std::fabs(v);
+    if (!(a < 448.f)) return sgn | 0x7Eu;
+    if (a < 0.015625f) return sgn | (uint8_t)std::nearbyint(a * 512.f);
+    int e;
+    const float fr = std::frexp(a, &e);
+    int q = (int)std::nearbyint((fr * 2.f - 1.f) * 8.f);
+    e -= 1;
+    if (q == 8) { q = 0; e += 1; }
+    const int code = ((e + 7) << 3) | q;
+    return sgn | (uint8_t)(code > 0x7E ? 0x7E : code);
+}
+static float host_f16_to_float(uint16_t h) { _Float16 x; memcpy(&x, &h, 2); return (float)x; }
+static uint32_t f8_scale_code(float maxhi, int* a_out) {
+    int a = 0;
+    if (maxhi > 0.f) {
+        while (maxhi * std::ldexp(1.f, a) > 448.f) a--;
+        while (maxhi * std::ldexp(1.f, a + 1) <= 448.f && a < 60) a++;
+    }
+    *a_out = a;
+    return (uint32_t)(127 - (a + SP_F8_XLO_LOG2));
+}
 extern "C" {
+
+int64_t sz_nn_split_stream_f8_bytes(int32_t n_blocks) {
+    const int64_t e = sz_nn_split_stream_elems(n_blocks);
+    return e < 0 ? e : e * 2 + 4 * 256;
+}
+int sz_nn_pack_split_stream_f8(const float* w_in, int32_t cin_real, int32_t ksize, int32_t conv, int32_t n_blocks, void* stream_v) {
+    if (!w_in || !stream_v || n_blocks < 0 || 1 + 2 * n_blocks > NN_MAX_CONVS_SPLIT || conv < 0 || conv > 1 + 2 * n_blocks) return SZ_ERR_INVALID;
+    if ((ksize == 1) != (conv == 1 + 2 * n_blocks) || (ksize != 1 && ksize != 3)) return SZ_ERR_INVALID;
+    if (conv == 0) return pack_split_stream_impl(w_in, cin_real, ksize, conv, (uint16_t*)stream_v, true);
+    if (cin_real <= 0 || cin_real > 256) return SZ_ERR_INVALID;
+    const int taps = ksize * ksize;
+    const size_t ks0 = 36 + (size_t)(conv - 1) * 72;
+    const float wscale = (float)(1 << SP_WSCALE_LOG2);
+    auto W = [&](int co, int ci, int t) -> float { return ci < cin_real ? w_in[((size_t)co * cin_real + ci) * taps + t] * wscale : 0.f; };
+    float maxhi = 0.f;
+    for (size_t i = 0; i < (size_t)256 * cin_real * taps; i++) maxhi = std::fmax(maxhi, std::fabs(host_f16_to_float(ElemF16::from_float(w_in[i] * wscale))));
+    int a;
+    const uint32_t code = f8_scale_code(maxhi, &a);
+    const float sh = std::ldexp(1.f, a), sl = std::ldexp(1.f, a + SP_F8_XLO_LOG2);
+    uint16_t* s16 = (uint16_t*)stream_v;
+    uint8_t* s8 = (uint8_t*)stream_v;
+    for (int t = 0; t < taps; t++)
+        for (int m = 0; m < 4; m++) {
+            const size_t ks = ks0 + (size_t)t * 8 + 2 * m;
+            for (int h = 0; h < 2; h++)
+                for (int tile = 0; tile < 16; tile++)
+                    for (int l = 0; l < 64; l++) {
+                        const int co = tile * 16 + (l & 15);
+                        const size_t u4 = ks * SP_KSTEP_U4 + (size_t)h * 1024 + (size_t)tile * 64 + l;
+                        for (int e = 0; e < 8; e++) s16[u4 * 8 + e] = ElemF16::from_float(W(co, 64 * m + 32 * h + 8 * (l >> 4) + e, t));
+                        for (int e = 0; e < 16; e++) {
+                            const float v = W(co, 64 * m + 16 * (l >> 4) + e, t), hi = host_f16_to_float(ElemF16::from_float(v));
+                            s8[(u4 + SP_KSTEP_U4) * 16 + e] = h == 0 ? host_e4m3(hi * sh) : host_e4m3((v - hi) * sl);
+                        }
+                    }
+        }
+    ((uint32_t*)(s8 + sz_nn_split_stream_elems(n_blocks) * 2))[conv] = code;
+    return SZ_OK;
+}
+int64_t sz_nn_split_head_f8_bytes(void) { return (int64_t)SP_HEAD_F8_U4 * 16 + 16; }
+int sz_nn_pack_split_head_f8(const float* w_in, void* out_v) {
+    if (!w_in || !out_v) return SZ_ERR_INVALID;
+    const float wscale = (float)(1 << SP_WSCALE_LOG2);
+    auto W = [&](int co, int ci) -> float { return co < 73 ? w_in[(size_t)co * 256 + ci] * wscale : 0.f; };
+    float maxhi = 0.f;
+    for (int i = 0; i < 73 * 256; i++) maxhi = std::fmax(maxhi, std::fabs(host_f16_to_float(ElemF16::from_float(w_in[i] * wscale))));
+    int a;
+    const uint32_t code = f8_scale_code(maxhi, &a);
+    const float sh = std::ldexp(1.f, a), sl = std::ldexp(1.f, a + SP_F8_XLO_LOG2);
+    uint16_t* o16 = (uint16_t*)out_v;
+    uint8_t* o8 = (uint8_t*)out_v;
+    for (int m = 0; m < 4; m++)
+        for (int tile = 0; tile < 5; tile++)
+            for (int l = 0; l < 64; l++) {
+                const int co = tile * 16 + (l & 15);
+                for (int p = 0; p < 2; p++)
+                    for (int e = 0; e < 8; e++) o16[((((size_t)m * 4 + p) * 5 + tile) * 64 + l) * 8 + e] = ElemF16::from_float(W(co, 64 * m + 32 * p + 8 * (l >> 4) + e));
+                for (int e = 0; e < 16; e++) {
+                    const float v = W(co, 64 * m + 16 * (l >> 4) + e), hi = host_f16_to_float(ElemF16::from_float(v));
+                    o8[((((size_t)m * 4 + 2) * 5 + tile) * 64 + l) * 16 + e] = host_e4m3(hi * sh);
+                    o8[((((size_t)m * 4 + 3) * 5 + tile) * 64 + l) * 16 + e] = host_e4m3((v - hi) * sl);
+                }
+            }
+    memset(o8 + (size_t)SP_HEAD_F8_U4 * 16, 0, 16);
+    memcpy(o8 + (size_t)SP_HEAD_F8_U4 * 16, &code, 4);
+    return SZ_OK;
+}
 
 static int pack_split_head_impl(const float* w_in, uint16_t* out, bool f16);
 int sz_nn_pack_split_head(const float* w_in, uint16_t* out) { return pack_split_head_impl(w_in, out, false); }
@@ -777,6 +1097,9 @@
 #define SPLIT_ATTR16(W, H) HIPCHK(hipFuncSetAttribute((const void*)k_tower_split<W, 0, H, ElemF16>, hipFuncAttributeMaxDynamicSharedMemorySize, SplitGeom<W>::LDS_BYTES))
         SPLIT_ATTR16(1, false); SPLIT_ATTR16(2, false); SPLIT_ATTR16(1, true); SPLIT_ATTR16(2, true);
 #undef SPLIT_ATTR16
+#define SPLIT_ATTR8(W, M, H) HIPCHK(hipFuncSetAttribute((const void*)k_tower_split<W, M, H, ElemF16F8>, hipFuncAttributeMaxDynamicSharedMemorySize, SplitGeom<W>::LDS_BYTES))
+        SPLIT_ATTR8(1, 0, false); SPLIT_ATTR8(2, 0, false); SPLIT_ATTR8(1, 0, true); SPLIT_ATTR8(2, 0, true); SPLIT_ATTR8(2, 1, false);
+#undef SPLIT_ATTR8
         attr_set = true;
     }
     const int n_cu = device_cus();
@@ -790,7 +1113,14 @@
                                                      (const uint4*)w_stream, bias, out, n_boards, n_blocks, (int)flags, ST, hp)
 #define SPLIT_LAUNCH16(W, H) hipLaunchKernelGGL((k_tower_split<W, 0, H, ElemF16>), grid, dim3(256), SplitGeom<W>::LDS_BYTES, (hipStream_t)stream, (const uint16_t*)planes, \
                                                   (const uint4*)w_stream, bias, out, n_boards, n_blocks, (int)flags, (unsigned long long*)nullptr, hp)
-    if (flags & SZ_NN_F16) {
+#define SPLIT_LAUNCH8(W, M, H, ST) hipLaunchKernelGGL((k_tower_split<W, M, H, ElemF16F8>), grid, dim3(256), SplitGeom<W>::LDS_BYTES, (hipStream_t)stream, \
+                                                      (const uint16_t*)planes, (const uint4*)w_stream, bias, out, n_boards, n_blocks, (int)flags, ST, hp)
+    if (flags & SZ_NN_SPLIT_F8) {
+        if (heads) { if (one) SPLIT_LAUNCH8(1, 0, true, (unsigned long long*)nullptr); else SPLIT_LAUNCH8(2, 0, true, (unsigned long long*)nullptr); }
+        else if (one) SPLIT_LAUNCH8(1, 0, false, (unsigned long long*)nullptr);
+        else if (g_split_stamps) SPLIT_LAUNCH8(2, 1, false, g_split_stamps);
+        else SPLIT_LAUNCH8(2, 0, false, (unsigned long long*)nullptr);
+    } else if (flags & SZ_NN_F16) {
         if (heads) { if (one) SPLIT_LAUNCH16(1, true); else SPLIT_LAUNCH16(2, true); }
         else { if (one) SPLIT_LAUNCH16(1, false); else SPLIT_LAUNCH16(2, false); }
     } else if (heads) {
@@ -803,6 +1133,7 @@
     else SPLIT_LAUNCH(2, 1, false, g_split_stamps);
 #undef SPLIT_LAUNCH
 #undef SPLIT_LAUNCH16
+#undef SPLIT_LAUNCH8
     HIPCHK(hipGetLastError());
     return SZ_OK;
 }
diff --git a/sigma-zero_amd/fastnet.py b/sigma-zero_amd/fastnet.py
--- a/sigma-zero_amd/fastnet.py
+++ b/sigma-zero_amd/fastnet.py
@@ -212,10 +212,11 @@
 
 class SplitPolicyNet:
 
-    def __init__(self, model, device=None, operands="bf16"):
+    def __init__(self, model, device=None, operands="f16f8"):
         model = model.eval()
-        assert operands in ("bf16", "fp16")
-        self.operands, self.f16 = operands, operands == "fp16"
+        assert operands in ("f16f8", "bf16", "fp16")
+        self.operands, self.f8 = operands, operands == "f16f8"
+        self.f16 = operands == "fp16" or self.f8
         if device is None:
             pdev = next(model.parameters()).device
             device = pdev if pdev.type == "cuda" else torch.device("cuda", torch.cuda.current_device())
@@ -231,21 +232,32 @@
             convs.append(_fold_bn(blk.conv2.weight, blk.bn2))
         self.n_blocks = len(model.resnet_blocks)
         L = N.lib()
-        stream = np.zeros(int(L.sz_nn_split_stream_elems(self.n_blocks)), dtype=np.uint16)
+        if self.f8:
+            stream = np.zeros(int(L.sz_nn_split_stream_f8_bytes(self.n_blocks)), dtype=np.uint8)
+        else:
+            stream = np.zeros(int(L.sz_nn_split_stream_elems(self.n_blocks)), dtype=np.uint16)
         wp1, bp1 = _fold_bn(model.conv_p1.weight, model.p_norm1)
         for k, (w, b) in enumerate(convs + [(wp1, bp1)]):
             wk = w.contiguous().cpu().float().numpy()
             assert wk.shape[0] == 256 and wk.shape[2] == wk.shape[3] == (1 if k == len(convs) else 3)
-            N.check((L.sz_nn_pack_split_stream_f16 if self.f16 else L.sz_nn_pack_split_stream)(wk.ctypes.data_as(C.c_void_p), wk.shape[1], wk.shape[2], k,
-                                                                                             stream.ctypes.data_as(C.c_void_p)), "sz_nn_pack_split_stream")
-        self._wstream = torch.from_numpy(stream.view(np.int16)).to(dev)
+            if self.f8:
+                N.check(L.sz_nn_pack_split_stream_f8(wk.ctypes.data_as(C.c_void_p), wk.shape[1], wk.shape[2], k, self.n_blocks, stream.ctypes.data_as(C.c_void_p)),
+                        "sz_nn_pack_split_stream_f8")
+            else:
+                N.check((L.sz_nn_pack_split_stream_f16 if self.f16 else L.sz_nn_pack_split_stream)(wk.ctypes.data_as(C.c_void_p), wk.shape[1], wk.shape[2], k,
+                                                                                                 stream.ctypes.data_as(C.c_void_p)), "sz_nn_pack_split_stream")
+        self._wstream = torch.from_numpy(stream.view(np.int8 if self.f8 else np.int16)).to(dev)
         self._bias = (torch.stack([b for _, b in convs] + [bp1]).float() * (1024.0 if self.f16 else 1.0)).contiguous().to(dev)
-        self._eflag = N.SZ_NN_F16 if self.f16 else 0
+        self._eflag = N.SZ_NN_SPLIT_F8 if self.f8 else N.SZ_NN_F16 if self.f16 else 0
         self.force_wgb = 0
         wp2 = model.conv_p2.weight.detach().view(73, 256).contiguous().cpu().float().numpy()
-        p2 = np.zeros(8 * 2 * 5 * 64 * 8, dtype=np.uint16)
-        N.check((L.sz_nn_pack_split_head_f16 if self.f16 else L.sz_nn_pack_split_head)(wp2.ctypes.data_as(C.c_void_p), p2.ctypes.data_as(C.c_void_p)), "sz_nn_pack_split_head")
-        self._wp2 = torch.from_numpy(p2.view(np.int16)).to(dev)
+        if self.f8:
+            p2 = np.zeros(int(L.sz_nn_split_head_f8_bytes()), dtype=np.uint8)
+            N.check(L.sz_nn_pack_split_head_f8(wp2.ctypes.data_as(C.c_void_p), p2.ctypes.data_as(C.c_void_p)), "sz_nn_pack_split_head_f8")
+        else:
+            p2 = np.zeros(8 * 2 * 5 * 64 * 8, dtype=np.uint16)
+            N.check((L.sz_nn_pack_split_head_f16 if self.f16 else L.sz_nn_pack_split_head)(wp2.ctypes.data_as(C.c_void_p), p2.ctypes.data_as(C.c_void_p)), "sz_nn_pack_split_head")
+        self._wp2 = torch.from_numpy(p2.view(np.int8 if self.f8 else np.int16)).to(dev)
         self.fused_heads = True
         self._hbuf, self._hcap = None, 0
         self.h_wp1, self.h_bp1 = wp1.view(256, 256).t().contiguous().to(dev), bp1.to(dev)
```
